# jjfiv/fastrank

Measured on AMD Instinct MI355X. Metric: coordinate-ascent NDCG@10 evals/sec on MSLR-WEB30K shape, higher is better.
Workload: dtype f64; 1 GPU; synthetic MSLR-WEB30K shape: 3800000 docs x 136 features x 31000 queries, coordinate ascent NDCG@10, 32 restarts/GPU x 25 steps/coord (configs[2]); restarts_total=32, parallelism=restart-sharded x1 (dataset replicated), launcher=single process

## Files before the change

fastrank_amd/csrc/capi.cpp:

```cpp
#include <atomic>
#include <limits>
#include <chrono>
#include <cstdio>
#include <cstdlib>
#include <cstring>
#include <fstream>

#include "../../include/fastrank.h"
#include "host.hpp"
#include "loader.hpp"
#include "explain_host.hpp"
#include "lambdamart.hpp"
#include "rf_train.hpp"

using fr::FrError;
using frjson::Value;

struct CDataset {
    std::shared_ptr<fr::DatasetView> view;
};
struct CModel {
    fr::Model actual;
};
struct CQRel {
// ... 1224 lines not shown
        auto holder = std::make_unique<FrTrainer>();
        holder->t0 = std::chrono::steady_clock::now();
        holder->t = std::make_unique<fr::CATrainer>(ds.view, std::move(ev), rq.ca, restart_begin, restart_end);
        holder->core = ds.view->core;
        h = holder.release();
    });
    if (st) {
        if (error_out) *error_out = st; else free((void*)st);
        return nullptr;
    }
    return h;
}

void* fr_ca_begin_query_shard(const void* train_request_json, const CDataset* dataset, uint64_t total_queries,
                              fr_allreduce_sum_fn allreduce, void* ctx, const void** error_out) {
    if (error_out) *error_out = nullptr;
    FrTrainer* h = nullptr;
    const void* st = status_call([&]() {
        const CDataset& ds = require_dataset(dataset);
        ParsedRequest rq = parse_train_request(accept_str("train_request_json", train_request_json));
        if (rq.learner != Learner::CoordinateAscent) fr::fail_str("fr_ca_begin_query_shard: only CoordinateAscent");
        if (!allreduce) fr::fail_str("fr_ca_begin_query_shard: allreduce callback is null!");
        std::lock_guard<std::mutex> lk(api_mu_of(ds));
        fr::Evaluator ev = fr::make_evaluator(*ds.view, rq.measure, rq.has_qrel ? &rq.qrel : nullptr);
        if (total_queries == 0) fr::fail_str("assertion failed: !data.queries().is_empty()");
        fr::QueryShard shard;
        shard.total_queries = total_queries;
        shard.allreduce = [allreduce, ctx](double* v, size_t n) {
            if (allreduce(ctx, v, n) != 0) fr::fail_str("query-shard allreduce callback failed");
        };
        auto holder = std::make_unique<FrTrainer>();
        holder->t0 = std::chrono::steady_clock::now();
        holder->t = std::make_unique<fr::CATrainer>(ds.view, std::move(ev), rq.ca, 0u, rq.ca.num_restarts, std::move(shard));
        holder->core = ds.view->core;
        h = holder.release();
    });
    if (st) {
        if (error_out) *error_out = st; else free((void*)st);
        return nullptr;
    }
    return h;
}

const void* fr_ca_step(void* trainer, uint64_t max_ticks, uint64_t* ticks_done, int* finished) {
    return status_call([&]() {
        if (!trainer) fr::fail_str("trainer pointer is null!");
        FrTrainer* h = (FrTrainer*)trainer;
        std::lock_guard<std::mutex> lk(h->core->api_mu);
        uint64_t n = 0;
        const bool alive = h->t->run(max_ticks, &n);
        if (ticks_done) *ticks_done = n;
        if (finished) *finished = (!alive || h->t->done()) ? 1 : 0;
    });
}

const void* fr_ca_state(void* trainer) {
    return json_call([&]() {
        if (!trainer) fr::fail_str("trainer pointer is null!");
        FrTrainer* h = (FrTrainer*)trainer;
        std::lock_guard<std::mutex> lk(h->core->api_mu);
        h->t->stats().seconds = std::chrono::duration<double>(std::chrono::steady_clock::now() - h->t0).count();
        Value o = Value::object();
        o.set("restarts", restarts_to_json(h->t->results()));
        o.set("stats", stats_to_json(h->t->stats()));
        o.set("finished", Value::boolean(h->t->done()));
        return frjson::dump(o);
    });
}

void fr_ca_free(void* trainer) { delete (FrTrainer*)trainer; }

const void* fr_ca_capture(void* trainer, int on) {
    return status_call([&]() {
        if (!trainer) fr::fail_str("trainer pointer is null!");
        FrTrainer* h = (FrTrainer*)trainer;
        std::lock_guard<std::mutex> lk(h->core->api_mu);
        h->t->capture(on != 0);
        if (!on) h->capture_blob.clear();
    });
}

const void* fr_ca_capture_take(void* trainer, const void* table, void* out, size_t out_bytes) {
    return json_call([&]() {
        if (!trainer) fr::fail_str("trainer pointer is null!");
        FrTrainer* h = (FrTrainer*)trainer;
        std::lock_guard<std::mutex> lk(h->core->api_mu);
        Value o = Value::object();
        if (table) {
            const std::string name = accept_str("table", table);
            if (name != "blob") fr::fail_str("fr_ca_capture_take: no table named " + name);
            if (out_bytes != h->capture_blob.size() || (!out && out_bytes))
                fr::fail_str("fr_ca_capture_take: the blob holds " + std::to_string(h->capture_blob.size()) + " bytes, the buffer " + std::to_string(out_bytes));
            if (out_bytes) std::memcpy(out, h->capture_blob.data(), out_bytes);
            o.set("bytes", Value::uint(out_bytes));
            h->capture_blob.clear();
            h->capture_blob.shrink_to_fit();
            return frjson::dump(o);
        }
        std::vector<frdev::LsCapture> log;
        h->t->take_capture(&log);
        std::vector<unsigned char>& blob = h->capture_blob;
        blob.clear();
        auto put = [&blob](const auto& v) {
            using T = typename std::remove_reference_t<decltype(v)>::value_type;
            blob.resize((blob.size() + 7) & ~size_t(7));
            Value r = Value::object();
            r.set("off", Value::uint(blob.size()));
            r.set("n", Value::uint(v.size()));
            const size_t at = blob.size();
            blob.resize(at + v.size() * sizeof(T));
            if (!v.empty()) std::memcpy(blob.data() + at, v.data(), v.size() * sizeof(T));
            return r;
        };
        Value events = Value::array();
        for (const frdev::LsCapture& e : log) {
            Value ev = Value::object();
            if (e.store) {
                ev.set("type", Value::string("store"));
                ev.set("slot", Value::sint(e.slot));
                ev.set("v", put(e.v));
                events.push(std::move(ev));
                continue;
            }
            static const char* const kinds[] = {"topk", "rr", "fullrank"};
            ev.set("type", Value::string("tick"));
            ev.set("ctx", Value::sint(e.ctx));
            ev.set("kind", Value::string(kinds[e.kind]));
            ev.set("measure", Value::sint(e.measure));
            ev.set("depth", Value::sint(e.depth));
            Value groups = Value::array();
            for (const frdev::LineGroup& lg : e.groups) {
                Value g = Value::object();
                g.set("feature", Value::uint(lg.feature));
                g.set("weights", put(lg.weights));
                g.set("candidates", put(lg.candidates));
                g.set("resident_slot", Value::sint(lg.resident_slot));
                g.set("resident_owner", Value::uint(lg.resident_owner));
                g.set("has_update", Value::boolean(lg.has_update));
                g.set("upd_feature", Value::uint(lg.upd_feature));
                g.set("params", put(std::vector<double>{lg.resident_norm, lg.resident_base_f, lg.resident_err, lg.upd_norm, lg.upd_base_f, lg.upd_cand}));
                groups.push(std::move(g));
            }
            ev.set("groups", std::move(groups));
            ev.set("gorder", put(e.gorder));
            ev.set("nverify", Value::uint(e.nverify));
            ev.set("approx", Value::boolean(e.approx));
            ev.set("resident", Value::boolean(e.resident));
            ev.set("ready", Value::boolean(e.ready));
            Value inst = Value::object();
            if (e.kind == 0) {
                inst.set("k", Value::sint(e.kbucket));
                inst.set("xs_used", Value::sint(e.xs_used));
                inst.set("xs_pinned", Value::boolean(e.xs_pinned));
            } else {
                inst.set("classes", put(e.classes));
            }
            inst.set("dup", Value::boolean(e.dup));
            ev.set("inst", std::move(inst));
            ev.set("redo", put(e.redo));
            ev.set("redo_groups", Value::uint(e.redo_groups));
            ev.set("means", put(e.means));
            ev.set("nq", Value::uint(e.nq));
            ev.set("ldm", Value::uint(e.ldm));
            ev.set("np", Value::uint(e.np));
            ev.set("has_matrix", Value::boolean(e.has_matrix));
            ev.set("matrix", put(e.matrix));
            ev.set("res_slots", put(e.res_slots));
            ev.set("res", put(e.res));
            events.push(std::move(ev));
        }
        o.set("events", std::move(events));
        o.set("bytes", Value::uint(blob.size()));
        return frjson::dump(o);
    });
}

const CResult* fr_select_model(const void* restarts_json, int output_ensemble) {
    return c_call<CModel>([&]() {
        std::vector<fr::RestartResult> hist = restarts_from_json_text(accept_str("restarts_json", restarts_json));
        std::stable_sort(hist.begin(), hist.end(),
                         [](const fr::RestartResult& a, const fr::RestartResult& b) { return a.restart_id < b.restart_id; });
        return new_model([&] { return fr::ca_select(hist, output_ensemble != 0); });
    });
}

const void* fr_last_train_stats(void) {
    return json_call([&]() {
        std::lock_guard<std::mutex> slk(g_stats_mu);
        Value o = stats_to_json(g_last_stats);
        if (!g_last_per_device.empty()) {
            Value a = Value::array();
            for (const fr::TrainStats& st : g_last_per_device) a.push(stats_to_json(st));
            o.set("per_device", std::move(a));
        }
        if (!g_last_lambdamart.is_null()) o.set("lambdamart", g_last_lambdamart);
        return frjson::dump(o);
    });
}

const void* fr_debug_tree_plan(void) {
    return json_call([&]() {
        const frdev::TreePlan p = frdev::last_tree_plan();
        Value o = Value::object();
        if (p.path == frdev::TreePlan::NONE) {
            o.set("path", Value::null());
            return frjson::dump(o);
        }
        o.set("path", Value::string(p.path == frdev::TreePlan::RANK ? "rank" : p.path == frdev::TreePlan::LDS ? "lds" : "l2"));
        o.set("cache_hit", Value::boolean(p.cache_hit));
        if (p.path == frdev::TreePlan::LDS) o.set("docs", Value::uint(p.docs)), o.set("parts", Value::uint(p.parts));
        if (p.path == frdev::TreePlan::L2) o.set("rows_in_lds", Value::boolean(p.rows_in_lds));
        if (p.path == frdev::TreePlan::RANK) o.set("nslots", Value::uint(p.nslots)), o.set("nrounds", Value::uint(p.nrounds));
        if (p.path != frdev::TreePlan::L2) {
            Value a = Value::array();
            for (const auto& b : p.batches) {
                Value pair = Value::array();
                pair.push(Value::uint(b.first)), pair.push(Value::uint(b.second));
                a.push(std::move(pair));
            }
            o.set("batches", std::move(a));
        }
        return frjson::dump(o);
    });
}

const void* fr_predict_scores_dense(const CModel* model, const CDataset* dataset, double* out, size_t out_len) {
    return status_call([&]() {
        const CModel& m = require_model(model);
        const CDataset& ds = require_dataset(dataset);
        std::lock_guard<std::mutex> lk(api_mu_of(ds));
        fr::DatasetView& view = *ds.view;
        if (view.instances.empty()) return;
        frdev::DeviceDataset& dev = view.device();
        fr::score_model(view, m.actual);
        std::string err;
        if (!dev.download_scores(0, out, out_len, &err)) fr::fail_str(err);
    });
}

namespace {

frdev::ExDocs explain_docs(fr::DatasetView& view) {
    frdev::DeviceDataset::TileForm tf;
    std::string err;
    if (!view.device().tile_form(&tf, &err)) fr::fail_str(err);
    if (tf.nonfinite) fr::fail_str("explain: the dataset holds inf or NaN feature values");
    frdev::ExDocs docs;
    docs.xb = tf.xb, docs.dq = (uint32_t)tf.dq, docs.d = (uint32_t)tf.d, docs.device = tf.device;
    docs.pos.reserve(tf.n), docs.ids.reserve(tf.n);
    for (size_t p = 0; p < tf.np; p++)
        if (tf.perm_host[p] != 0xFFFFFFFFu) docs.pos.push_back((uint32_t)p), docs.ids.push_back(tf.perm_host[p]);
    return docs;
}

size_t explain_budget() {
    const size_t free_b = frdev::device_free_bytes(), margin = (size_t)256 << 20;
    size_t budget = free_b > margin ? free_b - margin : 0;
    if (free_b == 0) budget = std::numeric_limits<size_t>::max();
    if (const char* e = std::getenv("FR_EXPLAIN_MAX_BYTES")) budget = std::min<size_t>(budget, (size_t)std::strtoull(e, nullptr, 10));
    return budget;
}

struct ExplainJob {
    fr::ExplainModel em;
    fr::ExplainPlan plan;
    frdev::ExDocs docs;
    std::vector<uint32_t> view_feats;
    std::vector<int64_t> out_col;
    frdev::ExTimes cover_t;
};

ExplainJob explain_prepare(const CModel& m, const CDataset& ds, const CDataset* bg) {
    ExplainJob job;
    job.em = fr::explain_model(m.actual);
    fr::DatasetView& view = *ds.view;
    fr::DatasetView& bview = bg ? *bg->view : view;
    if (bview.instances.empty()) fr::fail_str("explain: the background dataset holds no instance");
    job.view_feats = view.features;
    std::sort(job.view_feats.begin(), job.view_feats.end());
    if (view.instances.empty()) return job;
    job.docs = explain_docs(view);
    for (uint32_t f : job.em.feats) {
        const auto it = std::lower_bound(job.view_feats.begin(), job.view_feats.end(), f);
        const bool listed = it != job.view_feats.end() && *it == f;
        if (!listed && f < job.docs.d)
            fr::fail_str("explain: the model splits on feature " + std::to_string(f) + ", which the dataset's matrix holds but this feature sample does not list");
        job.out_col.push_back(listed ? (int64_t)(it - job.view_feats.begin()) : -1);
    }
    const frdev::ExWalk walk = fr::explain_walk(job.em);
    std::vector<uint32_t> counts;
    std::string err;
    if (&bview == &view) {
        if (!frdev::explain_covers(job.docs, walk, &counts, &job.cover_t, &err)) fr::fail_str(err);
    } else {
        const frdev::ExDocs bdocs = explain_docs(bview);
        if (bdocs.device != job.docs.device) fr::fail_str("explain: the background dataset lives on another device");
        if (!frdev::explain_covers(bdocs, walk, &counts, &job.cover_t, &err)) fr::fail_str(err);
    }
    job.plan = fr::explain_plan(job.em, counts, job.docs.d);
    return job;
}

Value explain_status(const ExplainJob& job, const frdev::ExTimes& t) {
    Value o = Value::object(), ids = Value::array(), sc = Value::array();
    for (uint32_t f : job.view_feats) ids.push(Value::uint(f));
    std::vector<uint64_t> counts(job.view_feats.size(), 0);
    for (size_t k = 0; k < job.out_col.size(); k++)
        if (job.out_col[k] >= 0) counts[(size_t)job.out_col[k]] = job.em.split_counts[k];
    for (uint64_t c : counts) sc.push(Value::uint(c));
    o.set("feature_ids", std::move(ids));
    o.set("split_counts", std::move(sc));
    o.set("expected_value", Value::number(job.plan.bias));
    o.set("trees", Value::uint(job.em.trees.size()));
    o.set("leaf_paths", Value::uint(job.plan.tab.value.size()));
    o.set("max_path", Value::uint(job.plan.tab.max_path));
    o.set("documents", Value::uint(job.docs.pos.size()));
    o.set("cover_ms", Value::number(job.cover_t.kernel_ms));
    o.set("kernel_ms", Value::number(t.kernel_ms));
    o.set("copy_ms", Value::number(t.copy_ms));
    return o;
}
// ... 717 lines not shown
```

fastrank_amd/csrc/device.hpp:

```cpp
#pragma once
#include <algorithm>
#include <cstddef>
#include <cstdint>
#include <memory>
#include <string>
#include <utility>
#include <vector>

#include "dataset_layout.hpp"

namespace frdev {

const char* path_env(const char* name);
inline const char* pricing_env(const char* name) {
#ifdef FR_PRICING
    return path_env(name);
#else
    (void)name;
    return nullptr;
#endif
}

enum Measure : int { M_NDCG = 0, M_AP = 1, M_RR = 2 };
constexpr int LM_OBJECTIVE_XENDCG = 3;

inline double resident_err_refresh(uint32_t d, double T) { return 1.1 * (double)(d + 1) * 0x1p-53 * T; }
inline double resident_err_update(double err, double norm, double T) { return 1.002 * err / norm + 8.0 * 0x1p-53 * T * (1.0 + 1e-6); }
inline double resident_eps_extra(double err, double norm, double T) { return 1.01 * err / norm + 10.0 * 0x1p-53 * T; }

enum : int {
    FLAG_NAN_SCORE = 1,
    FLAG_ACTUAL_GT_IDEAL = 2,
};

struct FlatTrees {
    std::vector<int32_t> fid, lhs, rhs;
    std::vector<double> split;
    std::vector<int32_t> root;
    std::vector<double> weight;
    bool raw_single = false;
};

struct TreePlan {
    enum Path { NONE, RANK, LDS, L2 };
    Path path = NONE;
    bool cache_hit = false;
    bool rows_in_lds = false;
    uint32_t docs = 0, parts = 0;
    uint32_t nslots = 0, nrounds = 0;
    std::vector<std::pair<uint32_t, uint32_t>> batches;
};
TreePlan last_tree_plan();

struct LineGroup {
    uint32_t feature = 0;
    std::vector<double> weights;
    std::vector<double> candidates;
    int resident_slot = -1;
    uint64_t resident_owner = 0;
    double resident_norm = 1.0, resident_base_f = 0.0, resident_err = 0.0;
    bool has_update = false;
    uint32_t upd_feature = 0;
    double upd_norm = 1.0, upd_base_f = 0.0, upd_cand = 0.0;
};

struct LsCapture {
    bool store = false;
    int slot = -1;
    std::vector<double> v;
    int ctx = 0, kind = 0, measure = 0;
    int64_t depth = 0;
    std::vector<LineGroup> groups;
    std::vector<uint32_t> gorder;
    size_t nverify = 0;
    bool approx = false, resident = false, ready = false;
    int kbucket = 0, xs_used = 0;
    bool xs_pinned = false, dup = false;
    std::vector<uint32_t> classes;
    std::vector<uint32_t> redo;
    uint32_t redo_groups = 0;
    std::vector<double> means;
    bool has_matrix = false;
    size_t nq = 0, ldm = 0, np = 0;
    std::vector<double> matrix;
    std::vector<int> res_slots;
    std::vector<double> res;
};

struct KernelStat {
    std::string name;
    uint64_t launches = 0;
    double total_ms = 0.0;
};

class DeviceDataset {
  public:
    static std::shared_ptr<DeviceDataset> create(const HostCSR& csr, std::string* err);
    static std::shared_ptr<DeviceDataset> create_view(const std::shared_ptr<DeviceDataset>& parent, const HostCSR& csr,
                                                      const std::vector<uint32_t>& parent_query, std::string* err);
    static std::shared_ptr<DeviceDataset> replicate(const std::shared_ptr<DeviceDataset>& src, int device, std::string* err);
    int device_ordinal() const;
    bool shares_parent_matrix() const;
    ~DeviceDataset();

    size_t n() const;
    size_t d() const;
    size_t nq() const;
    size_t max_query_len() const;
    size_t hbm_bytes() const;

    bool score_linear(size_t B, const double* weights, std::string* err);
    bool score_single_feature(uint32_t fid, double dir, std::string* err);
    bool score_trees(const FlatTrees& trees, std::string* err);
    bool ensemble_begin(std::string* err);
    bool ensemble_accumulate(double w, std::string* err);
    bool ensemble_finish(std::string* err);

    bool download_scores(size_t b, double* out_by_instance, size_t out_len, std::string* err);

    bool metric_from_scores(int measure, int64_t depth, const double* norms, size_t B,
                            bool want_rank, std::string* err);
    bool download_per_query(size_t B, double* out , std::string* err);
    bool download_rank(uint32_t* out_instance_ids , std::string* err);
    bool reduce_means(size_t ncols, double* out_means, std::string* err);
    void set_sums_only(bool on);
    bool subset_means_set(const std::vector<uint32_t>& a, const std::vector<uint32_t>& b, std::string* err);
    bool reduce_subset_means(double out_means[2], std::string* err);
    void subset_means_end();

    enum LsPath : int { LS_NONE = 0, LS_TOPK = 1, LS_FULLRANK = 2 };
    LsPath linesearch_path(int measure, int64_t depth) const;
    static constexpr int LINESEARCH_CONTEXTS = 4;
    struct LsCounts {
        unsigned long long pairs = 0, redone = 0;
    };
    bool linesearch_submit(int ctx, int measure, int64_t depth, const double* norms, const std::vector<LineGroup>& groups,
                           std::string* err);
    bool linesearch_collect(int ctx, std::vector<double>* means, LsCounts* counts, std::string* err);
    bool linesearch(int measure, int64_t depth, const double* norms, const std::vector<LineGroup>& groups,
                    std::vector<double>* means, LsCounts* counts, std::string* err);
    uint64_t resident_reserve(size_t slots, std::string* err);
    bool resident_store_from_scores(uint64_t owner, size_t slot, size_t b, std::string* err, const double* v = nullptr);
    void capture_enable(bool on);
    void capture_note_store(size_t slot, const double* v);
    void capture_take(std::vector<LsCapture>* out);
    const std::vector<double>& column_absmax() const;
    unsigned long long exact_fallbacks() const;
    void routing_counters(unsigned long long* exact_groups, unsigned long long* redo_entries) const;
    void chain_counters(unsigned long long* runs, unsigned long long* visits, unsigned long long* ranked_on = nullptr,
                        unsigned long long* ranked_off = nullptr) const;
    void audit_counters(unsigned long long* values, unsigned long long* mismatches) const;
    bool download_last_matrix(std::vector<double>* out, size_t* ldm, std::string* err);

    struct RfActive { uint32_t tree, key, n; };
    struct RfCand { double position, importance; uint32_t ids_i, flags, pos_l, pos_r; double sum_l, sum_r; };
    struct RfSplit { int32_t fslot; uint32_t pos, left, right; };
    bool rf_set_presence(const uint32_t* bits_by_instance, size_t words, size_t n_instances, std::string* err);
    bool rf_begin(const std::vector<uint32_t>& root_off, const std::vector<uint32_t>& root_ids, uint32_t nf,
                  const std::vector<uint32_t>& feats, std::string* err, const uint32_t* positions = nullptr,
                  bool lambda_targets = false);
    bool rf_positions(const std::vector<uint32_t>& root_ids, uint32_t* positions , std::string* err);
    bool rf_root_outputs(std::vector<double>* out, std::string* err);
    bool rf_level(const std::vector<RfActive>& active, const std::vector<uint32_t>& slot_of_key, uint32_t k, int method,
                  uint32_t min_leaf, std::vector<RfCand>* cands, std::vector<float>* label_minmax, std::string* err);
    bool rf_split(const std::vector<RfSplit>& splits, std::vector<double>* child_out, std::string* err);
    void rf_end();
    size_t rf_bytes_per_item() const { return 41; }

    struct LambdaPass {
        const unsigned char* query_flags = nullptr;
        bool flags_unchanged = false;
        uint32_t truncation_level = 0;
        bool lambda_norm = false;
        int objective = 0;
        uint64_t xe_key = 0;
    };
    bool lambda_gradients(const double* norms, int64_t depth, double sigma, const LambdaPass& pass, std::string* err);
    bool lambda_download_positions(std::vector<double>* lambda, std::vector<double>* weight, std::string* err);
    bool lambda_download(double* lambda_by_instance, double* weight_by_instance, size_t out_len, std::string* err,
                         const unsigned char* query_flags = nullptr);

    bool dart_begin(size_t rows, uint64_t* cache_bytes, std::string* err);
    bool dart_fill(size_t row, const double* leaf_values, size_t n_leaves, std::string* err);
    bool dart_rescore(const double* weights, size_t n_weights, const uint32_t* trees, size_t n_trees, std::string* err);
    bool dart_download_row(size_t row, uint16_t* out_by_instance, size_t out_len, std::string* err);
    void dart_end();

    struct HistNode { uint32_t slot, begin, end; };
    struct HistSplit { uint32_t begin, end, fslot, edge, nl; };
    struct HistSub { uint32_t parent, small, large; };
    struct HistBounds { double lo, hi; };
    struct HistSearch {
        uint32_t min_leaf; bool newton; int s_l, s_w; double lambda_l2, min_sum_hessian, min_split_gain; bool monotone;
        double lambda_l1 = 0.0, max_delta_step = 0.0, path_smooth = 0.0;
        bool reg() const { return lambda_l1 != 0.0 || max_delta_step != 0.0 || path_smooth != 0.0; }
    };
    struct HistRegNode { double lo, hi, parent; uint32_t has_parent, pad; };
    struct HistCand { double imp; long long ql, qtot, wl, wtot; uint32_t edge, nl, valid, fi; };
    bool hist_bins(const uint32_t* positions, size_t n, const std::vector<uint32_t>& feats, uint32_t k, bool* built, std::string* err);
    bool hist_edges(std::vector<float>* edges, std::vector<uint32_t>* nedges, std::string* err);
    bool hist_download_bins(uint8_t* out , size_t len, std::string* err);
    bool hist_sample(const unsigned char* query_flags, uint32_t n_t, const uint32_t* fsel, size_t f_t, std::string* err,
                     bool keep_queries = false);
    bool hist_goss(const double* lam_list, uint32_t n_top, double p, double amp, uint64_t tree_key, uint32_t* n_g, uint64_t* tau,
                   std::string* err);
    bool hist_goss_download(uint32_t* list, uint8_t* top, size_t len, std::string* err);
    bool hist_quantise(const double* lam_list, const double* wt_list, int* s_l, int* s_w, bool* all_zero, std::string* err);
    bool hist_quantq(uint32_t bits, uint64_t tree_key, int* d, int* d_w, std::string* err);
    bool hist_quantq_download(int32_t* q, uint32_t* w, size_t len, std::string* err);
    bool hist_root_download(uint32_t* cnt, long long* sum, long long* wsum, size_t cells, std::string* err);
    bool hist_root(bool newton, std::string* err);
    bool hist_search(const std::vector<HistNode>& nodes, const HistSearch& how, const std::vector<HistBounds>* bounds,
                     std::vector<HistCand>* best, std::string* err, const std::vector<HistRegNode>* reg = nullptr);
    bool hist_monotone(const int* signs, size_t features, std::string* err);
    struct HistSymBest { double key; uint32_t edge, valid; };
    bool hist_search_symmetric(const std::vector<HistNode>& nodes, const HistSearch& how, std::vector<HistSymBest>* best, std::string* err);
    bool hist_symmetric_apply(const std::vector<HistNode>& nodes, const HistSearch& how, uint32_t fi, uint32_t edge, std::vector<HistCand>* out,
                              std::string* err);
    bool hist_split(const std::vector<HistSplit>& splits, const std::vector<HistNode>& builds, const std::vector<HistSub>& subs,
                    uint32_t next_slots, bool newton, std::string* err);
    bool hist_leaf_sums(const std::vector<HistNode>& leaves, std::vector<long long>* qw , std::string* err);
    void hist_end();
    bool hist_leaf_begin(uint32_t slots, const HistSearch& how, HistCand* root, std::string* err);
    static constexpr uint32_t HIST_NO_SLOT = 0xffffffffu;
    struct HistLeafStep { HistSplit split; uint32_t parent_slot, small_slot; bool search_lhs, search_rhs; HistBounds bounds[2] = {}; double parent_out = 0.0; };
    bool hist_leaf_step(const HistLeafStep& step, const HistSearch& how, HistCand pick[2], std::string* err);

    struct TileForm {
        const float* xb = nullptr;
        size_t np = 0, dq = 0, d = 0, n = 0;
        int device = 0;
        bool nonfinite = false;
        const uint32_t* perm_host = nullptr;
    };
    bool tile_form(TileForm* out, std::string* err);

    int take_flags();

    std::vector<std::pair<std::string, uint64_t>> debug_form_scalars() const;
// ... 39 lines not shown
```

fastrank_amd/csrc/device_dataset.inc:

```

static constexpr int LS_CONTEXTS = DeviceDataset::LINESEARCH_CONTEXTS;

static double fv_class_cost(int ci) {
    static const int sort_ce[] = {63, 191, 384, 543, 849, 1056}, merge_ce[] = {32, 80, 144, 192, 304, 336};
    const uint32_t nl = FV_CLASSES[ci].nl, pl = FV_CLASSES[ci].pl;
    const int ni = (int)nl / 16 - 1;
    uint32_t rounds = 0;
    while ((1u << rounds) < pl) rounds++;
    double c = 2.0 * nl + 2.0 * sort_ce[ni] + 5.0 * nl + (double)nl * pl;
    for (uint32_t r = 1; r <= rounds; r++) c += 5.0 * r * nl + 2.0 * merge_ce[ni];
    static const double lane_penalty[] = {1.0, 1.1, 1.25, 1.6, 2.0, 2.4};
    return c * pl * lane_penalty[rounds];
}

static int fv_class_of(uint32_t len) {
    static const bool pow2_only = [] {
        const char* e = frdev::pricing_env("FR_FV_CLASSES");
        return e != nullptr && std::strcmp(e, "pow2") == 0;
    }();
    int best = -1;
    double best_cost = 0.0;
    for (int ci = 0; ci < FV_NCLASSES; ci++) {
        const uint32_t nl = FV_CLASSES[ci].nl, pl = FV_CLASSES[ci].pl, npad = nl * pl;
        if (npad < len) continue;
        if (pow2_only && ((npad & (npad - 1)) != 0 || (nl != 64 && pl != 1))) continue;
        const double c = fv_class_cost(ci);
        if (best < 0 || c < best_cost) best = ci, best_cost = c;
    }
    return best < 0 ? FV_NCLASSES - 1 : best;
}

void fullrank_class_of(uint32_t len, uint32_t* nl, uint32_t* pl) {
    const int ci = fv_class_of(len > 2048 ? 2048u : len);
    *nl = FV_CLASSES[ci].nl;
    *pl = FV_CLASSES[ci].pl;
}

std::vector<SizeClass> fv_build_classes(const std::vector<uint32_t>& qlen, std::vector<uint32_t>* list) {
    std::vector<int> cls_of_len(2049, -1);
    return bucket_queries(qlen, [&](uint32_t len) {
        const uint32_t l = len > 2048 ? 2048 : len;
        if (cls_of_len[l] < 0) cls_of_len[l] = fv_class_of(l);
        return cls_of_len[l];
    }, list);
}

static_assert(WT == WALK_TILE && LS_KT == DCG_RANKS && IDX_INVALID == NO_DOCUMENT, "the kernels' constants are the host layout's (dataset_layout.hpp)");

struct DatasetDesc {
    size_t n = 0, d = 0, nq = 0, np = 0, dq = 0, maxlen = 0, nruns = 0;
    bool nonfinite = false;
    bool labels_small_int = false;
    std::vector<double> colmax;
    int verify_xs = 1;
    std::vector<uint32_t> perm_host;
    std::vector<uint32_t> qstart_h, qlen_h, qnpos_h, qnneg_h;
    std::vector<uint32_t> wt_start_h;
    size_t nwt = 0;
    std::vector<double> colstd;
    std::vector<uint8_t> colmode;
    std::vector<ColStats> colstats_h;
    uint32_t key_bits = 0, key_cls_bits = 0;
    uint64_t dup_groups = 0;
    std::vector<SizeClass> size_classes;
    std::vector<SizeClass> fv_classes;
    uint64_t relmask = 0;
    size_t ncls = 0, tablen = 0;
};

struct StreamSignal {
    std::mutex mu;
    std::condition_variable cv;
    bool done = false, ok = true;
    void set(bool good) {
        {
            std::lock_guard<std::mutex> lk(mu);
            if (!good) ok = false;
            done = true;
        }
        cv.notify_all();
    }
    bool wait() {
        std::unique_lock<std::mutex> lk(mu);
        cv.wait(lk, [&] { return done; });
        return ok;
    }
};

struct DeviceDataset::Impl : DatasetDesc {
    struct TickStage {
        size_t G = 0, dp = 0;
        size_t o_count = 0, o_gredo = 0, o_gthr = 0, o_gmode = 0, o_rank = 0, o_gfeat = 0, o_gncand = 0, o_slot = 0, o_updf = 0, o_gcand = 0, o_eps2 = 0, o_par = 0, o_gw = 0, total = 0;
    };
    enum LsKind { LSK_TOPK, LSK_RR, LSK_FV };
    struct LsCtx {
        hipStream_t stream = nullptr;
        PinnedBuf tick_h, tick_res;
        DevBuf<unsigned char> tick_d;
        DevBuf<double> M, means, partial;
        DevBuf<uint32_t> redo;
        DevBuf<int> flags;
        template <typename T> T* th(size_t off) { return reinterpret_cast<T*>(tick_h.p + off); }
        template <typename T> T* td(size_t off) { return reinterpret_cast<T*>(tick_d.p + off); }
        bool pending = false, approx = false;
        bool ready = false;
        LsKind kind = LSK_TOPK;
        TickStage ts;
        LSArgs a;
        RRArgs ra;
        FSArgs fsa;
        RMArgs rma;
        DevBuf<double> fv_rows;
        size_t ldm = 0, maxc = 0, lds = 0;
        int64_t depth = 0;
        int measure = 0;
        int xs_used = 1;
        bool xs_pinned = false;
        bool audit = false;
        std::vector<LineGroup> agroups;
        unsigned redo_grid = 512, redo_grid_used = 512;
        size_t nverify = 0;
        std::vector<uint32_t> gorder, gredo_h;
        std::vector<int> gslot;
        std::vector<LineGroup> pgroups;
        std::vector<double> exact_means;
        LsCounts counts;
        bool resident = false, dup = false;
        int kbucket = 0;
        std::vector<LineGroup> cgroups;
    };
    LsCtx ls[LS_CONTEXTS + 1];
    hipEvent_t res_ready = nullptr;
    bool res_ready_set = false;
    const double* last_M = nullptr;
    DevBuf<uint32_t> sub_idx;
    DevBuf<double> sub_partial, sub_means;
    uint32_t sub_na = 0, sub_nb = 0;
    bool ls_submit(LsCtx& c, int path, int measure, int64_t depth, const double* norms, const std::vector<LineGroup>& groups,
                   std::string* err);
    struct LsTick { const std::vector<LineGroup>& groups; const double* norms; size_t nV; bool resident, any_update; };
    bool submit_topk(LsCtx& c, const LsTick& t, std::string* err);
    bool submit_rr(LsCtx& c, const LsTick& t, std::string* err);
    bool submit_fv(LsCtx& c, const LsTick& t, std::string* err);
    bool exact_instead(LsCtx& c, const LsTick& t, std::string* err);
    bool submit_queued(LsCtx& c, const LsTick& t, size_t nverify, std::string* err);
    bool ls_collect(LsCtx& c, std::vector<double>* means, std::string* err);
    bool topk_policy(LsCtx& c, uint32_t nredo, uint32_t nslices, std::string* err);
    bool ls_exact(LsCtx& c, int measure, int64_t depth, const double* norms, const std::vector<LineGroup>& groups, std::string* err);
    bool exact_kernels(const std::vector<LineGroup>& groups, int measure, int64_t depth, size_t maxc, double* M, int* flags, std::string* err);
    bool fr_audit(LsCtx& c, std::string* err);
    bool cap_on = false;
    std::vector<LsCapture> cap_log;
    const LsCtx* cap_outer = nullptr;
    bool capture_tick(LsCtx& c, const std::vector<double>& means, uint32_t nredo, std::string* err);
    bool ls_means(LsCtx& c, std::string* err);
    bool tick_begin(LsCtx& c, const std::vector<LineGroup>& groups, std::string* err);
    bool tick_upload(LsCtx& c, bool with_eps2, std::string* err);
    bool tick_finish(LsCtx& c, size_t ldm, std::vector<double>* means, uint32_t* nredo, std::string* err, uint32_t* npairs = nullptr,
                     std::vector<uint32_t>* by_group = nullptr);
    bool stage_resident(LsCtx& c, const std::vector<LineGroup>& groups, bool* any_update_out);
    bool compute_eps2(const std::vector<LineGroup>& groups, bool resident, uint32_t cls_bits, bool bare_admission = false, bool key_relative = false);
    double eps_gamma = 0.0;
    bool update_resident(LsCtx& c, size_t g_base, size_t ng, std::string* err);
    void flip_resident(const std::vector<LineGroup>& groups);
    bool redo_launch(LsCtx& c, uint32_t off, const uint32_t* count_dev, uint32_t n, std::string* err);
    FSArgs scores_args(const uint32_t* gfeat, const double* gw, const double* gcand, double* rows, int* flags, size_t gc) const;
    RMArgs rank_args(const double* rows, const uint32_t* gncand, double* M, int* flags, size_t gc, size_t ldm, int measure, int64_t depth) const;
    void topk_args(LsCtx& c, size_t G) const;
    RRArgs rr_args(LsCtx& c, size_t G) const;
    FVArgs fv_args(LsCtx& c, size_t G, uint32_t cls_bits, uint32_t dup_bits) const;
    int device = 0;
    hipStream_t stream = nullptr;
    std::vector<double> eps2_host;
    DevBuf<double> res;
    std::vector<uint8_t> res_half;
    uint64_t res_owner = 0;
    LsPolicy pol;
    unsigned long long approx_pairs = 0, approx_redo = 0;
    unsigned long long approx_redo_entries = 0;
    unsigned long long chain_runs = 0, chain_visits = 0;
    unsigned long long audit_values = 0, audit_mismatches = 0;
    DevBuf<double> audit;
    DevBuf<unsigned long long> audit_cnt;
    DevBuf<int> audit_flags;
    unsigned long long exact_fallbacks = 0;
    std::shared_ptr<DeviceDataset> parent;
    DevBuf<uint32_t> run_lo;
    DevBuf<uint32_t> vtiles;
    size_t nvtiles = 0;
    PosMap posmap() const { return PosMap{nvtiles ? vtiles.p : nullptr, (uint32_t)nvtiles, (uint32_t)np}; }
    size_t pos_threads() const { return nvtiles ? nvtiles * 64 : np; }
    DevBuf<uint8_t> xslot;
    DevBuf<uint16_t> segtab;
    DevBuf<uint32_t> wt_start;
    DevBuf<uint32_t> run_wt0;
    DevBuf<uint8_t> wofs;
    DevBuf<uint32_t> wlist;
    size_t nwlist = 0;
    DevBuf<uint8_t> rslot;
    hipError_t open_streams(bool* at_event, StreamSignal* main_stream = nullptr);
    bool open_streams(std::string* err);
    static bool upload_tiles(Impl& m, const HostCSR& csr, bool timing, StreamSignal& main_stream, std::string* terr);
    bool build_order_tables(std::string* err);
    DevBuf<float> xcol;
    bool build_columns(std::string* err);
    DevBuf<uint16_t> gkey;
    DevBuf<float> xb, gain;
    DevBuf<double> gexp, disc;
    DevBuf<uint32_t> qstart, qlen, qtight, perm, rank, run_q0, run_q1, run_pos, run_docs, run_order, gcls, qlist;
    DevBuf<uint32_t> fv_qlist;
    DevBuf<uint32_t> qnpos, qnneg, sort_idx;
    DevBuf<double> sort_keys;
    DevBuf<double> termtab, rows;
    DevBuf<double> dcgtab;
    DevBuf<int> flags;
    DevBuf<unsigned long long> dbgc;
    DevBuf<double> scores, acc, weights, M, means, partial, norms, gw, gcand;
    DevBuf<uint32_t> gfeat, gncand;
    DevBuf<TreeNodeDev> nodes;
    DevBuf<int32_t> roots;
    DevBuf<double> tweights;
    struct RfState {
        DevBuf<uint32_t> roff, pos, node_of, feats, slot_of_key, act_tree, act_n, vals_a, vals_b;
        DevBuf<uint64_t> act_off, act_first, keys_a, keys_b;
        DevBuf<float> sg, sv, sg_o, sv_o, label, gain_r;
        DevBuf<unsigned char> temp;
        DevBuf<RfCandDev> cands;
        DevBuf<RfSplitDev> splits;
        DevBuf<double> child;
        std::vector<uint32_t> roff_h;
        std::vector<uint32_t> pos_of_id;
        std::mutex pos_mu;
        uint32_t T = 0, nf = 0, total = 0;
        uint32_t A = 0;
        uint64_t items = 0, node_items = 0;
        bool sorted_in_b = false;
        uint64_t prev_items = 0;
        uint32_t prev_A = 0;
        DevBuf<uint32_t> act_tree_o, act_n_o;
        DevBuf<uint32_t> pres;
        uint32_t pw = 0;
        DevBuf<uint64_t> act_off_o;
        DevBuf<uint64_t> tile_first_o;
        DevBuf<uint32_t> tile_cnt;
        DevBuf<unsigned char> side, side_r;
        std::vector<uint32_t> prev_act_n;
        uint32_t splits_for_A = 0;
        const float* targets = nullptr;
    } rf;
    void rf_args(RFArgs& a);
    struct LmState {
        bool built = false;
        DevBuf<uint32_t> off, pos, qorder;
        DevBuf<double> lam, wt;
        DevBuf<float> target;
        DevBuf<unsigned char> slab;
        uint32_t n_lds = 0, max_len = 0;
        std::vector<uint32_t> order_h, qsel_h;
        uint32_t sel_long = 0;
        bool qsel_valid = false;
        DevBuf<uint32_t> qsel;
        DevBuf<double> asum;
    } lm;
    bool lm_build(std::string* err);
    struct DartState {
        DevBuf<uint16_t> leaf;
        DevBuf<double> vals, w;
        DevBuf<uint32_t> voff, trees;
        DevBuf<int> bad;
        std::vector<double> vals_h, w_h;
        std::vector<uint32_t> voff_h, trees_h;
        size_t rows = 0, filled = 0, stride = 0;
    } dart;
    struct HistState {
        uint32_t k = 0, n = 0, F = 0;
        uint32_t nt = 0, Ft = 0;
        bool q_sampled = false, f_sampled = false, qof_built = false, qof_ok = false;
        DevBuf<uint32_t> qof, root, fsel, total;
        DevBuf<uint8_t> qflag;
        bool g_on = false;
        uint32_t ng = 0;
// ... 1012 lines not shown
    const size_t ldm = c.ldm;
    if (!c.tick_res.ensure((ldm + mean_tail_words(ldm)) * sizeof(double), err)) return false;
    return launch_means(c.M.p, ldm, ldm, m.nq, m.sums_only, c.partial, c.means, c.stream, err, c.td<unsigned long long>(c.ts.o_count),
                        c.flags.p, reinterpret_cast<double*>(c.tick_res.p), c.kind == LSK_TOPK ? c.td<uint32_t>(c.ts.o_gredo) : nullptr);
}

bool DeviceDataset::Impl::tick_finish(LsCtx& c, size_t ldm, std::vector<double>* means, uint32_t* nredo, std::string* err,
                                      uint32_t* npairs, std::vector<uint32_t>* by_group) {
    Impl& m = *this;
    const size_t tail = ldm * sizeof(double);
    hipStream_t st = c.stream;
    FR_HIP(hipStreamSynchronize(st));
    means->resize(ldm);
    std::memcpy(means->data(), c.tick_res.p, tail);
    unsigned long long words[2] = {0, 0};
    std::memcpy(words, c.tick_res.p + tail, sizeof(words));
    *nredo = (uint32_t)words[0];
    if (npairs) *npairs = (uint32_t)(words[0] >> 32);
    if (by_group) {
        by_group->resize(2 * (ldm / 64));
        std::memcpy(by_group->data(), c.tick_res.p + tail + 16, 2 * (ldm / 64) * sizeof(uint32_t));
    }
    const int v = (int)(unsigned int)words[1];
    if (v) {
        m.host_flags |= v;
        FR_HIP(hipMemsetAsync(c.flags.p, 0, sizeof(int), st));
        FR_HIP(hipStreamSynchronize(st));
    }
    return true;
}
bool DeviceDataset::Impl::stage_resident(LsCtx& c, const std::vector<LineGroup>& groups, bool* any_update_out) {
    Impl& m = *this;
    const TickStage& ts = c.ts;
    LSArgs& a = c.a;
    const size_t G = groups.size();
    bool resident = G > 0, any_update = false;
    for (const LineGroup& lg : groups) {
        resident = resident && lg.resident_owner == m.res_owner && m.res_owner != 0 && lg.resident_slot >= 0 &&
                   (size_t)lg.resident_slot < m.res_half.size();
        any_update = any_update || lg.has_update;
    }
    a.res_cur = m.res.p;
    a.np = (uint32_t)m.np;
    a.rs_slot = nullptr;
    a.rs_par = nullptr;
    a.rs_updf = nullptr;
    a.xcol = m.xcol.p;
    if (resident) {
        int32_t* rs_slot = c.th<int32_t>(ts.o_slot);
        double* rs_par = c.th<double>(ts.o_par);
        uint32_t* rs_updf = c.th<uint32_t>(ts.o_updf);
        for (size_t g = 0; g < G; g++) {
            const LineGroup& lg = groups[g];
            rs_slot[g] = (int32_t)(lg.resident_slot * 2 + m.res_half[lg.resident_slot]);
            rs_par[g * 6 + 0] = 1.0 / lg.resident_norm;
            rs_par[g * 6 + 1] = lg.resident_base_f;
            rs_par[g * 6 + 2] = lg.has_update ? 1.0 : 0.0;
            rs_par[g * 6 + 3] = 1.0 / lg.upd_norm;
            rs_par[g * 6 + 4] = lg.upd_base_f;
            rs_par[g * 6 + 5] = lg.upd_cand;
            rs_updf[g] = lg.upd_feature;
        }
        a.rs_slot = c.td<int32_t>(ts.o_slot);
        a.rs_par = c.td<double>(ts.o_par);
        a.rs_updf = c.td<uint32_t>(ts.o_updf);
    }
    *any_update_out = any_update;
    return resident;
}

bool DeviceDataset::Impl::compute_eps2(const std::vector<LineGroup>& groups, bool resident, uint32_t cls_bits, bool bare_admission, bool key_relative) {
    Impl& m = *this;
    const size_t G = groups.size();
    std::vector<double>& eps2 = m.eps2_host;
    eps2.assign(G * 64, 0.0);
    const double dfac = (key_relative && resident) ? (double)(m.d + 2) : 2.5 * (double)(m.d + 1);
    const double gamma = (dfac * std::ldexp(1.0, -53) + (bare_admission ? 3.0 : 2.0) * std::ldexp(1.0, (int)cls_bits - 52)) * (1.0 + 1e-6);
    bool ok = true;
    for (size_t g = 0; g < G; g++) {
        const LineGroup& lg = groups[g];
        double T = 0.0;
        for (size_t j = 0; j < m.d; j++)
            if (j != lg.feature) T += std::fabs(lg.weights[j]) * m.colmax[j];
        double extra = 0.0;
        if (resident) {
            T += std::fabs(lg.resident_base_f) * m.colmax[lg.feature];
            extra = resident_eps_extra(lg.resident_err, lg.resident_norm, T);
            if (!(lg.resident_norm > 0.0) || !(extra < 1e290)) ok = false;
        }
        for (size_t c = 0; c < lg.candidates.size(); c++) {
            const double Tc = T + std::fabs(lg.candidates[c]) * m.colmax[lg.feature];
            if (!(Tc < 1e290)) ok = false;
            const double floor_abs = 1e-300 + std::fabs(lg.candidates[c]) * std::ldexp(1.0, (int)cls_bits - 1070);
            eps2[g * 64 + c] = key_relative ? 2.0 * (gamma * 2.0 * T + extra + floor_abs) : 2.0 * (gamma * Tc + extra + floor_abs);
        }
    }
    m.eps_gamma = gamma;
    return ok;
}

bool DeviceDataset::Impl::update_resident(LsCtx& c, size_t g_base, size_t ng, std::string* err) {
    Impl& m = *this;
    LSArgs x = c.a;
    x.g_base = (uint32_t)g_base;
    x.posmap = m.posmap();
    {
        ProfScope ps("resident_update_kernel", c.stream);
        resident_update_kernel<<<dim3((unsigned)((m.pos_threads() + 255) / 256), (unsigned)ng), 256, 0, c.stream>>>(x);
    }
    FR_HIP(hipGetLastError());
    return true;
}


void DeviceDataset::Impl::flip_resident(const std::vector<LineGroup>& groups) {
    Impl& m = *this;
    std::vector<char> flipped(m.res_half.size(), 0);
    for (const LineGroup& lg : groups)
        if (lg.has_update && !flipped[lg.resident_slot]) {
            m.res_half[lg.resident_slot] ^= 1;
            flipped[lg.resident_slot] = 1;
        }
}

template <int K, int CT>
static void launch_linesearch(const LSArgs& a, unsigned nblocks, size_t lds, hipStream_t st) {
    linesearch_ndcg_kernel<K, CT, 16><<<dim3(nblocks), dim3(WAVE), lds, st>>>(a);
}

template <int K>
static void dispatch_ct(const LSArgs& a, unsigned nblocks, size_t maxc, size_t lds, hipStream_t st) {
    if (maxc <= 4) launch_linesearch<K, 4>(a, nblocks, lds, st);
    else if (maxc <= 16) launch_linesearch<K, 16>(a, nblocks, lds, st);
    else if (maxc <= 32) launch_linesearch<K, 32>(a, nblocks, lds, st);
    else if (maxc <= 51) launch_linesearch<K, 51>(a, nblocks, lds, st);
    else launch_linesearch<K, 64>(a, nblocks, lds, st);
}

static void dispatch_exact(const LSArgs& a, int64_t depth, unsigned nblocks, size_t maxc, size_t lds, hipStream_t st) {
    if (a.work_list != nullptr) {
        maxc = std::min<size_t>(maxc, 16);
        nblocks *= 4;
    }
    if (depth <= 5) dispatch_ct<5>(a, nblocks, maxc, lds, st);
    else if (depth <= 10) dispatch_ct<10>(a, nblocks, maxc, lds, st);
    else dispatch_ct<20>(a, nblocks, maxc, lds, st);
}

static unsigned redo_grid_env() {
    const char* e = frdev::path_env("FR_REDO_GRID");
    return e ? (unsigned)std::min<long>(std::max<long>(std::atol(e), 64), 1 << 20) : 0u;
}

template <int K>
static void launch_verify(const LSArgs& a, bool resident, bool dupk, int xs, unsigned nruns8, size_t G, size_t dp, size_t tab_lds_kt, hipStream_t st) {
    const size_t tab_lds = tab_lds_kt / (LS_KT + 1) * (K + 1);
    if (resident) {
        const dim3 grid((unsigned)(nruns8 * G));
        if (dupk) {
            if (xs <= 1) linesearch_verify_kernel<K, 1, true, 1, true><<<grid, dim3(WAVE), tab_lds, st>>>(a);
            else if (xs == 2) linesearch_verify_kernel<K, 1, true, 2, true><<<grid, dim3(WAVE), tab_lds, st>>>(a);
            else if (xs == 3 || K < 10) linesearch_verify_kernel<K, 1, true, 3, true><<<grid, dim3(WAVE), tab_lds, st>>>(a);
            else linesearch_verify_kernel<K, 1, true, (K < 10 ? 3 : 4), true><<<grid, dim3(WAVE), tab_lds, st>>>(a);
        } else if (xs <= 1) linesearch_verify_kernel<K, 1, true><<<grid, dim3(WAVE), tab_lds, st>>>(a);
        else if (xs == 2) linesearch_verify_kernel<K, 1, true, 2><<<grid, dim3(WAVE), tab_lds, st>>>(a);
        else if (xs == 3 || K < 10) linesearch_verify_kernel<K, 1, true, 3><<<grid, dim3(WAVE), tab_lds, st>>>(a);
        else linesearch_verify_kernel<K, 1, true, (K < 10 ? 3 : 4)><<<grid, dim3(WAVE), tab_lds, st>>>(a);
    } else {
        const dim3 grid((unsigned)(nruns8 * ((G + 1) / 2)));
        linesearch_verify_kernel<K, 2, false><<<grid, dim3(WAVE), 2 * dp * sizeof(double) + tab_lds, st>>>(a);
    }
}

uint64_t DeviceDataset::resident_reserve(size_t slots, std::string* err) {
    Impl& m = *impl_;
    std::lock_guard<std::mutex> lk(m.mu);
    if (!m.bind(err)) return 0;
    m.res_owner++;
    m.verify_xs = std::max(1, m.verify_xs - 1);
    m.res_half.clear();
    if (m.xcol.p == nullptr) {
        if (err) *err = "resident_reserve: the dataset has no column-major copy";
        return 0;
    }
    m.pol.reset(slots);
    {
        std::string* e2 = err;
        auto ensure = [&]() -> bool { return m.res.ensure(slots * 2 * m.np, e2); };
        if (!ensure()) return 0;
    }
    m.res_half.assign(slots, 0);
    if (m.xslot.p != nullptr) {
        std::string e2;
        if (m.rslot.ensure(slots * m.np, &e2)) {
            rslot_identity_kernel<<<dim3(1024), dim3(256), 0, m.stream>>>(m.rslot.p, m.wofs.p, m.np, slots * m.np);
            if (hipGetLastError() != hipSuccess) m.rslot.release();
        } else {
            (void)hipGetLastError();
        }
    }
    return m.res_owner;
}

bool DeviceDataset::resident_store_from_scores(uint64_t owner, size_t slot, size_t b, std::string* err, const double* v) {
    Impl& m = *impl_;
    std::lock_guard<std::mutex> lk(m.mu);
    if (err) err->clear();
    if (owner != m.res_owner) return false;
    if (!m.bind(err)) return false;
    if (slot >= m.res_half.size() || b >= m.scores_slots) {
        if (err) *err = "resident_store_from_scores: slot out of range";
        return false;
    }
    FR_HIP(hipMemcpyAsync(m.res.p + (slot * 2 + m.res_half[slot]) * m.np, m.scores.p + b * m.np, m.np * sizeof(double),
                          hipMemcpyDeviceToDevice, m.stream));
    FR_HIP(hipEventRecord(m.res_ready, m.stream));
    m.res_ready_set = true;
    m.pol.new_sums(slot);
    if (m.cap_on) {
        LsCapture e;
        e.store = true;
        e.slot = (int)slot;
        if (v) e.v.assign(v, v + m.d);
        m.cap_log.push_back(std::move(e));
    }
    return true;
}

void DeviceDataset::capture_enable(bool on) {
    std::lock_guard<std::mutex> lk(impl_->mu);
    impl_->cap_on = on;
    if (!on) impl_->cap_log.clear();
    for (Impl::LsCtx& c : impl_->ls) std::vector<LineGroup>().swap(c.cgroups);
}

void DeviceDataset::capture_note_store(size_t slot, const double* v) {
    std::lock_guard<std::mutex> lk(impl_->mu);
    if (!impl_->cap_on) return;
    LsCapture e;
    e.store = true;
    e.slot = (int)slot;
    e.v.assign(v, v + impl_->d);
    impl_->cap_log.push_back(std::move(e));
}

void DeviceDataset::capture_take(std::vector<LsCapture>* out) {
    std::lock_guard<std::mutex> lk(impl_->mu);
    out->clear();
    out->swap(impl_->cap_log);
}

const std::vector<double>& DeviceDataset::column_absmax() const { return impl_->colmax; }

void DeviceDataset::audit_counters(unsigned long long* values, unsigned long long* mismatches) const {
    std::lock_guard<std::mutex> lk(impl_->mu);
    *values = impl_->audit_values;
    *mismatches = impl_->audit_mismatches;
}

unsigned long long DeviceDataset::exact_fallbacks() const {
    std::lock_guard<std::mutex> lk(impl_->mu);
    return impl_->exact_fallbacks;
}

void DeviceDataset::chain_counters(unsigned long long* runs, unsigned long long* visits, unsigned long long* ranked_on,
                                   unsigned long long* ranked_off) const {
    std::lock_guard<std::mutex> lk(impl_->mu);
    *runs = impl_->chain_runs;
    *visits = impl_->chain_visits;
    if (ranked_on) *ranked_on = impl_->pol.rank_slots_on;
    if (ranked_off) *ranked_off = impl_->pol.rank_slots_off;
}

void DeviceDataset::routing_counters(unsigned long long* exact_groups, unsigned long long* redo_entries) const {
    std::lock_guard<std::mutex> lk(impl_->mu);
    *exact_groups = impl_->pol.exact_groups;
    *redo_entries = impl_->approx_redo_entries;
}

static void launch_scores(const FSArgs& a, size_t maxc, unsigned nblocks, size_t lds, hipStream_t st) {
    if (maxc <= 16) linesearch_scores_kernel<16, 16><<<dim3(nblocks), dim3(WAVE), lds, st>>>(a);
    else if (maxc <= 51) linesearch_scores_kernel<51, 16><<<dim3(nblocks), dim3(WAVE), lds, st>>>(a);
    else linesearch_scores_kernel<64, 16><<<dim3(nblocks), dim3(WAVE), lds, st>>>(a);
}

FSArgs DeviceDataset::Impl::scores_args(const uint32_t* gf, const double* w, const double* cand, double* rows, int* fl, size_t gc) const {
    FSArgs a{};
    a.xb = (const float4*)xb.p;
    a.run_pos = run_pos.p;
    a.run_docs = run_docs.p;
    a.run_order = run_order.p;
    a.gfeat = gf;
    a.gw = w;
    a.gcand = cand;
    a.rows = rows;
    a.flags = fl;
    a.dq = (uint32_t)dq;
    a.d = (uint32_t)d;
    a.nruns = (uint32_t)nruns;
    a.GC = (uint32_t)gc;
    a.np = (uint32_t)np;
    return a;
}

RMArgs DeviceDataset::Impl::rank_args(const double* rows, const uint32_t* gnc, double* out, int* fl, size_t gc, size_t ldm, int measure,
                                      int64_t depth) const {
    RMArgs a{};
    a.rows = rows;
    a.qstart = qstart.p;
    a.qlen = qlen.p;
    a.qnpos = qnpos.p;
    a.qnneg = qnneg.p;
    a.gcls = gcls.p;
    a.termtab = termtab.p;
    a.norms = norms.p;
    a.gncand = gnc;
    a.M = out;
    a.flags = fl;
    a.GC = (uint32_t)gc;
    a.np = (uint32_t)np;
// ... 256 lines not shown
            return false;
        }
        maxc = std::max(maxc, lg.candidates.size());
    }
    if (&c == &m.ls[LS_CONTEXTS]) c.stream = m.stream;
    c.kind = path == LS_TOPK ? LSK_TOPK : (measure == M_RR ? LSK_RR : LSK_FV);
    c.ldm = G * 64;
    c.maxc = maxc;
    c.depth = depth;
    c.measure = measure;
    c.approx = c.ready = false;
    c.resident = c.dup = false;
    c.kbucket = 0;
    c.nverify = 0;
    c.gorder.clear();
    c.counts = LsCounts{};
    if (m.cap_on) c.cgroups = groups_in;
    if (G == 0) {
        c.pending = true;
        return true;
    }
    const bool topk = c.kind == LSK_TOPK;
    if (topk) {
        if (m.nq * G >= (size_t(1) << 28)) {
            if (err) *err = "linesearch: too many (query, group) pairs for one launch";
            return false;
        }
        if (!c.M.ensure(m.nq * c.ldm, err) || !c.redo.ensure(m.nq * G, err)) return false;
    }
    const bool exact_only = std::getenv("FR_LS_EXACT") != nullptr;
    c.audit = std::getenv("FR_VERIFY_AUDIT") != nullptr;
    bool can_verify = !exact_only && m.colmax.size() == m.d;
    if (c.kind != LSK_RR) can_verify = can_verify && m.ncls <= 256;
    if (c.kind == LSK_FV)
        can_verify = can_verify && frdev::path_env("FR_FV_OFF") == nullptr && (measure == M_NDCG ? m.termtab.cap > 0 : m.ncls <= 31);
    if (!can_verify && !topk) return m.ls_exact(c, measure, depth, norms, groups_in, err);
    if (c.kind != LSK_RR) {
        if (!m.norms.ensure(m.nq, err)) return false;
        const uint64_t tok = groups_in[0].resident_owner;
        if (!(tok != 0 && tok == m.norms_token && norms == m.norms_token_ptr)) {
            const bool fresh = !(m.norms_cache.size() == m.nq && std::memcmp(m.norms_cache.data(), norms, m.nq * sizeof(double)) == 0);
            if (!m.upload_norms(norms, err)) return false;
            if (fresh) FR_HIP(hipStreamSynchronize(m.stream));
            m.norms_token = tok;
            m.norms_token_ptr = norms;
        }
    }
    size_t nV = can_verify ? G : 0;
    const std::vector<LineGroup>* gp = &groups_in;
    if (topk && can_verify && m.res_owner != 0) {
        const size_t nE = m.pol.route(G, [&](size_t g) { return groups_in[g].resident_owner == m.res_owner ? (long)groups_in[g].resident_slot : -1L; });
        nV = G - nE;
        if (nE > 0 && nV > 0) {
            c.gorder.resize(G);
            size_t iv = 0, ie = nV;
            for (size_t g = 0; g < G; g++) c.gorder[m.pol.routed[g] ? ie++ : iv++] = (uint32_t)g;
            c.pgroups.clear();
            for (size_t k = 0; k < G; k++) c.pgroups.push_back(groups_in[c.gorder[k]]);
            gp = &c.pgroups;
        }
    }
    if (topk && nV == 0) m.exact_fallbacks++;
    if (!m.tick_begin(c, *gp, err)) return false;
    c.a = LSArgs{};
    LsTick t{*gp, norms, nV, false, false};
    t.resident = m.stage_resident(c, t.groups, &t.any_update);
    c.resident = t.resident;
    switch (c.kind) {
        case LSK_TOPK: return m.submit_topk(c, t, err);
        case LSK_RR: return m.submit_rr(c, t, err);
        case LSK_FV: return m.submit_fv(c, t, err);
    }
    return false;
}

bool DeviceDataset::Impl::submit_queued(LsCtx& c, const LsTick& t, size_t nverify, std::string* err) {
    Impl& m = *this;
    const size_t G = t.groups.size();
    const bool approx = nverify > 0;
    FR_HIP(hipGetLastError());
    if (!m.ls_means(c, err)) return false;
    if (t.resident) m.flip_resident(t.groups);
    c.gslot.assign(G, -1);
    if (t.resident)
        for (size_t k = 0; k < G; k++) c.gslot[k] = t.groups[k].resident_slot;
    c.agroups.clear();
    if (c.audit && approx && c.kind != LSK_TOPK) c.agroups.assign(t.groups.begin(), t.groups.end());
    c.approx = approx;
    c.nverify = nverify;
    c.pending = true;
    return true;
}

bool DeviceDataset::Impl::exact_instead(LsCtx& c, const LsTick& t, std::string* err) {
    Impl& m = *this;
    if (t.resident && t.any_update) {
        if (!m.update_resident(c, 0, t.groups.size(), err)) return false;
        m.flip_resident(t.groups);
    }
    FR_HIP(hipStreamSynchronize(c.stream));
    return m.ls_exact(c, c.measure, c.depth, t.norms, t.groups, err);
}

bool DeviceDataset::Impl::submit_topk(LsCtx& c, const LsTick& t, std::string* err) {
    Impl& m = *this;
    const std::vector<LineGroup>& groups = t.groups;
    const size_t G = groups.size(), dp = m.dq * 4, nruns8 = ((m.nruns + 7) / 8) * 8, maxc = c.maxc;
    const int64_t depth = c.depth;
    const bool resident = t.resident;
    const TickStage& ts = c.ts;
    size_t nV = t.nV;
    LSArgs& a = c.a;
    m.topk_args(c, G);
    static const int ls_debug = [] {
        const char* dbg = frdev::pricing_env("FR_LS_DEBUG");
        return dbg ? atoi(dbg) : 0;
    }();
    LS_DEBUG_SET(a, ls_debug);
    if (LS_DEBUG(a) & 16) FR_HIP(hipMemsetAsync(m.dbgc.p, 0, 4 * sizeof(unsigned long long), c.stream));
    if (nruns8 * G > 0x7fffffffull) {
        if (err) *err = "linesearch: grid too large";
        return false;
    }
    c.lds = 2 * dp * sizeof(double);
    bool approx = nV > 0 && (LS_DEBUG(a) & ~3) == 0;
    if (approx) approx = m.compute_eps2(groups, resident, m.key_bits, true, true);
    a.gamma = m.eps_gamma;
    const size_t tab_lds = (m.ncls + 1) * (size_t)(LS_KT + 1) * sizeof(double);
    if (approx && !resident && 2 * dp * sizeof(double) + tab_lds + 2 * (WAVE + 4) * sizeof(uint4) > 64 * 1024) approx = false;
    if (!approx && nV > 0) {
        m.exact_fallbacks++;
        nV = 0;
    }
    size_t nrank = 0;
    a.xslot = nullptr;
    if (approx && resident && m.xslot.p != nullptr && m.rslot.p != nullptr && m.colstd.size() == m.d) {
        static const double kappa = [] {
            const char* e = frdev::pricing_env("FR_ORDER_KAPPA");
            return e ? std::atof(e) : 1.0;
        }();
        static const unsigned period = [] {
            const char* e = frdev::pricing_env("FR_RANK_PERIOD");
            return e ? (unsigned)std::max(1, std::atoi(e)) : 16u;
        }();
        double* gthr = c.th<double>(ts.o_gthr);
        uint32_t* gmode = c.th<uint32_t>(ts.o_gmode);
        for (size_t g = 0; g < nV; g++) {
            gthr[g] = order_threshold(groups[g].weights, m.colstd, groups[g].feature, kappa);
            gmode[g] = m.colmode[groups[g].feature];
        }
        int32_t* rank = c.th<int32_t>(ts.o_rank);
        nrank = m.pol.plan_rank_refresh(nV, [&](size_t g) { return (size_t)groups[g].resident_slot; }, [&](size_t g) { return groups[g].has_update; },
                                        period, m.res_half, rank, rank + G);
        a.xslot = m.xslot.p;
        a.rslot = m.rslot.p;
        a.gthr = c.td<double>(ts.o_gthr);
        a.gmode = c.td<uint32_t>(ts.o_gmode);
    }
    if (!m.tick_upload(c, approx, err)) return false;
    if (!approx) {
        if (resident && t.any_update && !m.update_resident(c, 0, G, err)) return false;
        {
            ProfScope ps("linesearch_ndcg_kernel", c.stream);
            dispatch_exact(a, depth, (unsigned)(nruns8 * G), maxc, c.lds, c.stream);
        }
        return m.submit_queued(c, t, 0, err);
    }
    if (nrank > 0) {
        ProfScope ps("rslot_kernel", c.stream);
        const uint32_t* wl = m.nwlist ? m.wlist.p : nullptr;
        const unsigned nw = (unsigned)(m.nwlist ? m.nwlist : m.nwt);
        rslot_kernel<<<dim3((nw + 3) / 4), 256, 0, c.stream>>>(m.res.p, c.td<int32_t>(ts.o_rank), c.td<int32_t>(ts.o_rank) + G, (uint32_t)nrank,
                                                              a.rs_par, a.rs_updf, m.xcol.p, m.segtab.p, m.wt_start.p, wl, nw, (uint32_t)m.np, m.rslot.p);
        FR_HIP(hipGetLastError());
        if (c.audit) {
            if (!m.audit_cnt.ensure(1, err)) return false;
            FR_HIP(hipMemsetAsync(m.audit_cnt.p, 0, sizeof(unsigned long long), c.stream));
            const int32_t* rk = c.th<int32_t>(ts.o_rank);
            for (size_t k = 0; k < nrank; k++)
                order_audit_kernel<<<dim3((nw + 3) / 4), 256, 0, c.stream>>>(m.rslot.p + (size_t)(rk[k] >> 1) * m.np, m.segtab.p, m.wt_start.p, wl, nw, m.audit_cnt.p);
            for (size_t g = 0; g < nV; g++)
                order_audit_kernel<<<dim3((nw + 3) / 4), 256, 0, c.stream>>>(m.xslot.p + (size_t)groups[g].feature * m.np, m.segtab.p, m.wt_start.p, wl, nw, m.audit_cnt.p);
            unsigned long long bad = 0;
            FR_HIP(hipMemcpyAsync(&bad, m.audit_cnt.p, sizeof(bad), hipMemcpyDeviceToHost, c.stream));
            FR_HIP(hipStreamSynchronize(c.stream));
            m.audit_mismatches += bad;
        }
    }
    const char* xs_e = frdev::path_env("FR_VERIFY_XS");
    const int xs = std::min(xs_e ? std::atoi(xs_e) : m.verify_xs, verify_xs_cap(depth));
    c.xs_used = xs;
    c.xs_pinned = xs_e != nullptr;
    a.eps2 = c.td<double>(ts.o_eps2);
    a.G = (uint32_t)nV;
    const bool dupk = resident && m.key_bits > m.key_cls_bits;
    c.dup = dupk;
    {
        ProfScope ps("linesearch_verify_kernel", c.stream);
        if (depth <= 5) launch_verify<5>(a, resident, dupk, xs, (unsigned)nruns8, nV, dp, tab_lds, c.stream), c.kbucket = 5;
        else if (depth <= 10) launch_verify<10>(a, resident, dupk, xs, (unsigned)nruns8, nV, dp, tab_lds, c.stream), c.kbucket = 10;
        else launch_verify<20>(a, resident, dupk, xs, (unsigned)nruns8, nV, dp, tab_lds, c.stream), c.kbucket = 20;
    }
    FR_HIP(hipGetLastError());
    a.slice_count = c.td<uint32_t>(ts.o_count) + 1;
    const unsigned redo_pin = redo_grid_env();
    c.redo_grid_used = redo_pin ? redo_pin : c.redo_grid;
    if (!m.redo_launch(c, 0, c.td<uint32_t>(ts.o_count), c.redo_grid_used, err)) return false;
    if (nV < G) {
        if (t.any_update && !m.update_resident(c, nV, G - nV, err)) return false;
        LSArgs x = a;
        x.work_list = nullptr;
        x.work_count = nullptr;
        x.g_base = (uint32_t)nV;
        x.G = (uint32_t)(G - nV);
        ProfScope ps("linesearch_ndcg_kernel", c.stream);
        dispatch_exact(x, depth, (unsigned)(nruns8 * (G - nV)), maxc, c.lds, c.stream);
    }
    return m.submit_queued(c, t, nV, err);
}

bool DeviceDataset::Impl::submit_rr(LsCtx& c, const LsTick& t, std::string* err) {
    Impl& m = *this;
    const size_t G = t.groups.size();
    if (!t.resident) return m.ls_exact(c, c.measure, c.depth, t.norms, t.groups, err);
    bool approx = m.compute_eps2(t.groups, true, 0);
    if (approx && m.pol.take_skip()) m.exact_fallbacks++, approx = false;
    if (!m.tick_upload(c, approx, err)) return false;
    if (!approx) return m.exact_instead(c, t, err);
    if (!c.M.ensure(m.nq * c.ldm, err) || !c.redo.ensure(m.nq * G, err)) return false;
    RRArgs& ra = c.ra;
    ra = m.rr_args(c, G);
    {
        ProfScope ps("rr_verify_kernel", c.stream);
        FR_HIP(hipFuncSetAttribute((const void*)rr_verify_kernel, hipFuncAttributeMaxDynamicSharedMemorySize, 128 * 1024));
        for (size_t ci = m.size_classes.size(); ci-- > 0;) {
            const auto& sc = m.size_classes[ci];
            ra.qlist = m.qlist.p + sc.offset;
            rr_verify_kernel<<<dim3((unsigned)sc.count, (unsigned)G), WAVE, (size_t)sc.npad * sizeof(uint4), c.stream>>>(ra);
        }
    }
    FR_HIP(hipGetLastError());
    const unsigned redo_pin = redo_grid_env();
    c.redo_grid_used = redo_pin ? redo_pin : RR_REDO_GRID;
    if (!m.redo_launch(c, 0, c.td<uint32_t>(c.ts.o_count), c.redo_grid_used, err)) return false;
    return m.submit_queued(c, t, G, err);
}

bool DeviceDataset::Impl::submit_fv(LsCtx& c, const LsTick& t, std::string* err) {
    Impl& m = *this;
    const size_t G = t.groups.size();
    uint32_t cls_bits = 0;
    while ((size_t(1) << cls_bits) < m.ncls + 1) cls_bits++;
    const uint32_t dup_bits = (m.key_bits > m.key_cls_bits && cls_bits + (m.key_bits - m.key_cls_bits) <= 20) ? m.key_bits - m.key_cls_bits : 0u;
    bool approx = m.compute_eps2(t.groups, t.resident, cls_bits + dup_bits);
    if (approx && m.pol.take_skip()) m.exact_fallbacks++, approx = false;
    if (!m.tick_upload(c, approx, err)) return false;
    if (!approx) return m.exact_instead(c, t, err);
    if (!c.M.ensure(m.nq * c.ldm, err) || !c.redo.ensure(m.nq * G, err)) return false;
    const size_t slot_rows = ((m.maxlen + 63) / 64 + 1) * 64;
    if (!c.fv_rows.ensure((size_t)FV_REDO_GRID * slot_rows * 64, err)) return false;
    FVArgs fa = m.fv_args(c, G, cls_bits, dup_bits);
    c.dup = dup_bits != 0;
    {
        static const bool per_class = frdev::pricing_env("FR_FV_PROFILE") != nullptr;
        ProfScope ps_all(per_class ? "fullrank_verify_all" : "fullrank_verify_kernel", c.stream);
        for (size_t ci = m.fv_classes.size(); ci-- > 0;) {
            const auto& sc = m.fv_classes[ci];
            static std::vector<std::string> names = [] {
                std::vector<std::string> v;
                for (int i = 0; i < FV_NCLASSES; i++) v.push_back("fullrank_verify_kernel<" + std::to_string(FV_CLASSES[i].nl) + "x" + std::to_string(FV_CLASSES[i].pl) + ">");
                return v;
            }();
            std::unique_ptr<ProfScope> ps(per_class ? new ProfScope(names[sc.npad].c_str(), c.stream) : nullptr);
            fa.qlist = m.fv_qlist.p + sc.offset;
            if (!fv_launch_class(fa, (int)sc.npad, (unsigned)sc.count, (unsigned)G, (unsigned)c.maxc, c.stream)) {
                if (err) *err = "fullrank_verify_kernel: no instantiation for this size class";
                return false;
            }
        }
    }
    FR_HIP(hipGetLastError());
    FSArgs& fs = c.fsa;
    fs = m.scores_args(fa.gfeat, fa.gw, fa.gcand, c.fv_rows.p, c.flags.p, G);
    fs.qstart = m.qstart.p;
    fs.qlen = m.qlen.p;
    fs.G = (uint32_t)G;
    fs.slot_rows = (uint32_t)slot_rows;
    RMArgs& rm = c.rma;
    rm = m.rank_args(c.fv_rows.p, fa.gncand, c.M.p, c.flags.p, G, c.ldm, c.measure, c.depth);
    rm.G = (uint32_t)G;
    rm.slot_rows = (uint32_t)slot_rows;
    c.redo_grid_used = FV_REDO_GRID;
    if (!m.redo_launch(c, 0, c.td<uint32_t>(c.ts.o_count), FV_REDO_GRID, err)) return false;
    return m.submit_queued(c, t, G, err);
}

bool DeviceDataset::Impl::ls_exact(LsCtx& c, int measure, int64_t depth, const double* norms, const std::vector<LineGroup>& groups,
                                   std::string* err) {
    Impl& m = *this;
    if (&c != &m.ls[LS_CONTEXTS]) {
        c.pgroups.assign(groups.begin(), groups.end());
        for (LineGroup& lg : c.pgroups) lg.has_update = false;
        LsCtx& l = m.ls[LS_CONTEXTS];
        m.cap_outer = &c;
        const bool done = m.ls_submit(l, LS_FULLRANK, measure, depth, norms, c.pgroups, err) && m.ls_collect(l, &c.exact_means, err);
        m.cap_outer = nullptr;
        if (!done) return false;
        c.counts = l.counts;
        c.ready = c.pending = true;
        return true;
    }
    const size_t G = groups.size(), ldm = G * 64;
    std::vector<double>& means = c.exact_means;
    means.assign(ldm, 0.0);
    if (!m.M.ensure(m.nq * ldm, err) || !m.norms.ensure(m.nq, err) || !m.means.ensure(ldm, err)) return false;
    if (!m.upload_norms(norms, err)) return false;
    if (!m.exact_kernels(groups, measure, depth, c.maxc, m.M.p, m.flags.p, err)) return false;
    if (!launch_means(m.M.p, ldm, ldm, m.nq, m.sums_only, m.partial, m.means, m.stream, err)) return false;
    FR_HIP(hipMemcpyAsync(means.data(), m.means.p, ldm * sizeof(double), hipMemcpyDeviceToHost, m.stream));
    m.last_ldm = ldm;
    m.last_cols = ldm;
    m.last_M = m.M.p;
    if (!m.pull_flags(err)) return false;
    c.ready = c.pending = true;
    return true;
}

bool DeviceDataset::Impl::exact_kernels(const std::vector<LineGroup>& groups, int measure, int64_t depth, size_t maxc, double* M,
                                        int* flags, std::string* err) {
    Impl& m = *this;
    const size_t G = groups.size(), dp = m.dq * 4, ldm = G * 64;
    const size_t row_bytes = 64 * sizeof(double);
    size_t budget = m.rows.bytes();
    if (G * m.np * row_bytes > budget) {
        size_t free_b = 0, total_b = 0;
        (void)hipMemGetInfo(&free_b, &total_b);
        budget = std::max<size_t>(size_t(1) << 30, (free_b + m.rows.bytes()) / 2);
    }
    size_t GC = std::max<size_t>(1, std::min<size_t>(G, budget / (m.np * row_bytes)));
    if (!m.rows.ensure(m.np * GC * 64, err) || !m.gfeat.ensure(GC, err) || !m.gncand.ensure(GC, err) || !m.gw.ensure(GC * dp, err) ||
        !m.gcand.ensure(GC * 64, err))
        return false;
    for (size_t g0 = 0; g0 < G; g0 += GC) {
        const size_t gc = std::min(GC, G - g0);
        std::vector<uint32_t> gfeat(gc), gncand(gc);
        std::vector<double> gw(gc * dp, 0.0), gcand(gc * 64, 0.0);
        for (size_t g = 0; g < gc; g++) {
            const LineGroup& lg = groups[g0 + g];
            gfeat[g] = lg.feature;
            gncand[g] = (uint32_t)lg.candidates.size();
            std::memcpy(&gw[g * dp], lg.weights.data(), m.d * sizeof(double));
            std::memcpy(&gcand[g * 64], lg.candidates.data(), lg.candidates.size() * sizeof(double));
        }
        FR_HIP(hipMemcpyAsync(m.gfeat.p, gfeat.data(), gc * sizeof(uint32_t), hipMemcpyHostToDevice, m.stream));
        FR_HIP(hipMemcpyAsync(m.gncand.p, gncand.data(), gc * sizeof(uint32_t), hipMemcpyHostToDevice, m.stream));
        FR_HIP(hipMemcpyAsync(m.gw.p, gw.data(), gc * dp * sizeof(double), hipMemcpyHostToDevice, m.stream));
        FR_HIP(hipMemcpyAsync(m.gcand.p, gcand.data(), gc * 64 * sizeof(double), hipMemcpyHostToDevice, m.stream));
        FR_HIP(hipStreamSynchronize(m.stream));
        {
            ProfScope ps("linesearch_scores_kernel", m.stream);
            const FSArgs fa = m.scores_args(m.gfeat.p, m.gw.p, m.gcand.p, m.rows.p, flags, gc);
            launch_scores(fa, maxc, (unsigned)(((m.nruns + 7) / 8) * 8 * gc), 2 * dp * sizeof(double), m.stream);
        }
        FR_HIP(hipGetLastError());
        RMArgs ra = m.rank_args(m.rows.p, m.gncand.p, M, flags, gc, ldm, measure, depth);
        ra.col0 = (uint32_t)(g0 * 64);
        {
            ProfScope ps("rank_metric_kernel", m.stream);
            FR_HIP(hipFuncSetAttribute((const void*)rank_metric_kernel, hipFuncAttributeMaxDynamicSharedMemorySize,
                                       128 * 1024));
            for (size_t ci = m.size_classes.size(); ci-- > 0;) {
                const auto& sc = m.size_classes[ci];
                ra.qlist = m.qlist.p + sc.offset;
                dim3 grid((unsigned)sc.count, (unsigned)gc);
                const unsigned waves = (measure != M_NDCG && measure != M_AP) ? 1u
                                       : sc.npad <= 128 ? 1u : (sc.npad <= 256 ? 2u : (sc.npad <= 512 ? 4u : 8u));
                rank_metric_kernel<<<grid, WAVE * waves, (size_t)sc.npad * 64, m.stream>>>(ra);
            }
        }
        FR_HIP(hipGetLastError());
    }
    return true;
}

bool DeviceDataset::Impl::ls_collect(LsCtx& c, std::vector<double>* means, std::string* err) {
    Impl& m = *this;
    c.pending = false;
    if (c.ready) {
        *means = c.exact_means;
        if (m.cap_on) return m.capture_tick(c, *means, 0, err);
        return true;
    }
    const size_t ldm = c.ldm, G = ldm / 64;
    means->assign(ldm, 0.0);
    if (G == 0) return true;
    uint32_t nredo = 0, nslices = 0;
    std::vector<uint32_t>& by_group = c.gredo_h;
    if (!m.tick_finish(c, ldm, means, &nredo, err, &nslices, c.kind == LSK_TOPK ? &by_group : nullptr)) return false;
    LSArgs& a = c.a;
    if (c.approx) {
        const size_t nV = c.nverify;
        m.approx_pairs += m.nq * nV;
        m.approx_redo += nredo;
        c.counts.pairs += m.nq * nV;
        c.counts.redone += nredo;
        const unsigned grid = c.redo_grid_used;
        uint32_t again = 0;
        if (nredo > grid &&
            (!m.redo_launch(c, grid, nullptr, nredo - grid, err) || !m.ls_means(c, err) || !m.tick_finish(c, ldm, means, &again, err, &nslices)))
            return false;
        switch (c.kind) {
            case LSK_TOPK:
                if (!m.topk_policy(c, nredo, nslices, err)) return false;
                break;
            default:
                m.pol.observe_skip(nredo, m.nq, G);
                if (c.audit && !m.fr_audit(c, err)) return false;
                break;
        }
    }
    if (!c.gorder.empty()) {
        std::vector<double> tmp(*means);
        for (size_t k = 0; k < G; k++) std::memcpy(means->data() + (size_t)c.gorder[k] * 64, tmp.data() + k * 64, 64 * sizeof(double));
    }
    m.last_ldm = ldm;
    m.last_cols = ldm;
    m.last_M = c.M.p;
    if (LS_DEBUG(a) & 16) {
        unsigned long long cnt[4];
        FR_HIP(hipMemcpyAsync(cnt, m.dbgc.p, sizeof(cnt), hipMemcpyDeviceToHost, c.stream));
        FR_HIP(hipStreamSynchronize(c.stream));
        fprintf(stderr, "[FR_LS_DEBUG] docs=%llu rows=%llu (%.3f of docs) batches=%llu insertion_rows=%llu\n", cnt[3], cnt[0],
                (double)cnt[0] / (double)cnt[3], cnt[1], cnt[2]);
    }
    if (m.cap_on) return m.capture_tick(c, *means, c.approx ? nredo : 0, err);
    return true;
}

bool DeviceDataset::Impl::capture_tick(LsCtx& c, const std::vector<double>& means, uint32_t nredo, std::string* err) {
    Impl& m = *this;
    const bool lockstep = &c == &m.ls[LS_CONTEXTS];
    if (c.ready && !lockstep) return true;
    const LsCtx& who = (lockstep && m.cap_outer) ? *m.cap_outer : c;
    if (who.cgroups.size() * 64 != c.ldm) return true;
    LsCapture e;
    e.ctx = (int)(&who - m.ls);
    e.kind = (int)c.kind;
    e.measure = c.measure;
    e.depth = c.depth;
    e.groups = who.cgroups;
    const size_t G = e.groups.size();
    e.gorder = c.gorder;
    if (e.gorder.empty())
        for (size_t g = 0; g < G; g++) e.gorder.push_back((uint32_t)g);
    e.nverify = c.approx ? c.nverify : 0;
    e.approx = c.approx;
    e.resident = who.resident;
    e.ready = c.ready;
    hipStream_t st = c.ready ? m.stream : c.stream;
    if (c.kind == LSK_TOPK) {
        e.kbucket = c.kbucket;
        e.xs_used = c.kbucket ? c.xs_used : 0;
        e.xs_pinned = c.kbucket ? c.xs_pinned : false;
    } else if (c.approx) {
        if (c.kind == LSK_FV)
            for (const auto& sc : m.fv_classes) e.classes.insert(e.classes.end(), {FV_CLASSES[sc.npad].nl, FV_CLASSES[sc.npad].pl, sc.count});
        else
            for (const auto& sc : m.size_classes) e.classes.insert(e.classes.end(), {sc.npad, 1u, sc.count});
    }
    e.dup = c.dup;
    e.redo_groups = (uint32_t)(c.kind == LSK_TOPK ? c.nverify : G);
    if (c.approx && nredo > 0) {
        e.redo.resize(nredo);
        FR_HIP(hipMemcpyAsync(e.redo.data(), c.redo.p, nredo * sizeof(uint32_t), hipMemcpyDeviceToHost, st));
    }
    e.means = means;
    e.nq = m.nq;
    e.ldm = G * 64;
    e.np = m.np;
    const double* M = c.ready ? m.M.p : c.M.p;
    e.has_matrix = M != nullptr;
    if (e.has_matrix) {
        e.matrix.resize(e.nq * e.ldm);
        FR_HIP(hipMemcpyAsync(e.matrix.data(), M, e.matrix.size() * sizeof(double), hipMemcpyDeviceToHost, st));
    }
    if (e.resident) {
        for (const LineGroup& lg : e.groups) e.res_slots.push_back(lg.resident_slot);
        std::sort(e.res_slots.begin(), e.res_slots.end());
        e.res_slots.erase(std::unique(e.res_slots.begin(), e.res_slots.end()), e.res_slots.end());
        e.res.resize(e.res_slots.size() * m.np);
        for (size_t i = 0; i < e.res_slots.size(); i++) {
            const size_t slot = (size_t)e.res_slots[i];
            FR_HIP(hipMemcpyAsync(e.res.data() + i * m.np, m.res.p + (slot * 2 + m.res_half[slot]) * m.np, m.np * sizeof(double), hipMemcpyDeviceToHost, st));
        }
    }
    FR_HIP(hipStreamSynchronize(st));
    m.cap_log.push_back(std::move(e));
    return true;
}

bool DeviceDataset::Impl::fr_audit(LsCtx& c, std::string* err) {
    Impl& m = *this;
    const size_t nel = m.nq * c.ldm;
    if (!m.audit.ensure(nel, err) || !m.audit_cnt.ensure(1, err) || !m.audit_flags.ensure(1, err)) return false;
    FR_HIP(hipMemsetAsync(m.audit.p, 0xFF, nel * sizeof(double), m.stream));
    size_t ncells = 0;
    for (size_t g = 0; g < c.agroups.size(); g++) {
        const size_t nc = c.agroups[g].candidates.size();
        ncells += m.nq * nc;
        if (nc < 64)
            FR_HIP(hipMemcpy2DAsync(m.audit.p + g * 64 + nc, c.ldm * sizeof(double), c.M.p + g * 64 + nc, c.ldm * sizeof(double),
                                    (64 - nc) * sizeof(double), m.nq, hipMemcpyDeviceToDevice, m.stream));
    }
    FR_HIP(hipMemsetAsync(m.audit_flags.p, 0, sizeof(int), m.stream));
    if (!m.exact_kernels(c.agroups, c.measure, c.depth, c.maxc, m.audit.p, m.audit_flags.p, err)) return false;
    FR_HIP(hipMemsetAsync(m.audit_cnt.p, 0, sizeof(unsigned long long), m.stream));
    audit_compare_kernel<<<dim3(1024), dim3(256), 0, m.stream>>>(m.audit.p, c.M.p, nel, m.audit_cnt.p);
    FR_HIP(hipGetLastError());
    unsigned long long bad = 0;
    FR_HIP(hipMemcpyAsync(&bad, m.audit_cnt.p, sizeof(bad), hipMemcpyDeviceToHost, m.stream));
    FR_HIP(hipStreamSynchronize(m.stream));
    m.audit_values += ncells;
    m.audit_mismatches += bad;
    return true;
}

bool DeviceDataset::Impl::topk_policy(LsCtx& c, uint32_t nredo, uint32_t nslices, std::string* err) {
    Impl& m = *this;
    const size_t ldm = c.ldm, G = ldm / 64, nV = c.nverify;
    const std::vector<uint32_t>& by_group = c.gredo_h;
    LSArgs& a = c.a;
    c.redo_grid = next_redo_grid(c.redo_grid, c.redo_grid_used, nredo);
    m.approx_redo_entries += nslices;
    for (size_t k = 0; k < nV; k++) m.chain_runs += by_group[G + k];
    m.chain_visits += (unsigned long long)m.n * nV;
    {
        static const double t_off = [] {
            const char* e = frdev::pricing_env("FR_RANK_OFF_BELOW");
            return e ? std::atof(e) : RANK_OFF_BELOW;
        }();
        static const double t_on = [] {
            const char* e = frdev::pricing_env("FR_RANK_ON_ABOVE");
            return e ? std::atof(e) : RANK_ON_ABOVE;
        }();
        m.pol.observe_chain(nV, [&](size_t k) { return (long)c.gslot[k]; }, [&](size_t k) { return by_group[G + k]; }, m.n, t_off, t_on);
    }
    if (c.audit) {
        const size_t nel = m.nq * ldm;
        if (!m.audit.ensure(nel, err) || !m.audit_cnt.ensure(1, err)) return false;
        FR_HIP(hipMemcpyAsync(m.audit.p, c.M.p, nel * sizeof(double), hipMemcpyDeviceToDevice, c.stream));
        LSArgs x = a;
        x.work_list = nullptr;
        x.work_count = nullptr;
        x.g_base = 0;
        x.G = (uint32_t)G;
        dispatch_exact(x, c.depth, (unsigned)(((m.nruns + 7) / 8) * 8 * G), c.maxc, c.lds, c.stream);
        FR_HIP(hipMemsetAsync(m.audit_cnt.p, 0, sizeof(unsigned long long), c.stream));
        audit_compare_kernel<<<dim3(1024), dim3(256), 0, c.stream>>>(m.audit.p, c.M.p, nel, m.audit_cnt.p);
        unsigned long long bad = 0;
        FR_HIP(hipMemcpyAsync(&bad, m.audit_cnt.p, sizeof(bad), hipMemcpyDeviceToHost, c.stream));
        FR_HIP(hipStreamSynchronize(c.stream));
        m.audit_values += nel;
        m.audit_mismatches += bad;
    }
    m.pol.observe_redo(nV, [&](size_t k) { return (long)c.gslot[k]; }, [&](size_t k) { return by_group[k]; }, m.nq, c.xs_used, verify_xs_cap(c.depth),
                       c.xs_pinned, LS_DEBUG(a), m.verify_xs);
    return true;
}

bool DeviceDataset::linesearch_submit(int ctx, int measure, int64_t depth, const double* norms, const std::vector<LineGroup>& groups,
                                      std::string* err) {
    Impl& m = *impl_;
    std::lock_guard<std::mutex> lk(m.mu);
    if (!m.bind(err)) return false;
    if (ctx < 0 || ctx >= LS_CONTEXTS || m.ls[ctx].pending) {
        if (err) *err = "linesearch_submit: no such context, or a submitted line search was not collected";
        return false;
    }
    return m.ls_submit(m.ls[ctx], linesearch_path(measure, depth), measure, depth, norms, groups, err);
}

bool DeviceDataset::linesearch_collect(int ctx, std::vector<double>* means, LsCounts* counts, std::string* err) {
    Impl& m = *impl_;
    std::lock_guard<std::mutex> lk(m.mu);
    if (!m.bind(err)) return false;
    if (ctx < 0 || ctx >= LS_CONTEXTS || !m.ls[ctx].pending) {
        if (err) *err = "linesearch_collect: nothing was submitted on this context";
        return false;
    }
    if (!m.ls_collect(m.ls[ctx], means, err)) return false;
    if (counts) *counts = m.ls[ctx].counts;
    return true;
}

bool DeviceDataset::linesearch(int measure, int64_t depth, const double* norms, const std::vector<LineGroup>& groups,
                               std::vector<double>* means, LsCounts* counts, std::string* err) {
    Impl& m = *impl_;
    std::lock_guard<std::mutex> lk(m.mu);
    if (!m.bind(err)) return false;
    const LsPath path = linesearch_path(measure, depth);
    Impl::LsCtx& c = m.ls[path == LS_TOPK ? 0 : LS_CONTEXTS];
    if (c.pending) {
        if (err) *err = "linesearch: context 0 busy (collect the submitted line search first)";
        return false;
    }
    if (!m.ls_submit(c, path, measure, depth, norms, groups, err) || !m.ls_collect(c, means, err)) return false;
    if (counts) *counts = c.counts;
    return true;
}





#include "train_rf.inc"
#include "train_lambda.inc"
#include "train_dart.inc"
#include "train_hist.inc"
```

fastrank_amd/csrc/kernels_linesearch.inc:

```
struct LSArgs {
    const float4* xb;
    const uint32_t* gcls;
    const double* dcgtab;
    const uint32_t* qstart;
    const uint32_t* qlen;
    const uint32_t* run_q0;
    const uint32_t* run_q1;
    const uint32_t* run_pos;
    const uint32_t* run_lo;
    const uint32_t* run_docs;
    const uint32_t* run_order;
    const uint32_t* wt_start;
    const uint32_t* run_wt0;
    const double* norms;
    const double* disc;
    const uint32_t* gfeat;
    const double* gw;
    const double* gcand;
    const uint32_t* gncand;
    double* M;
    int* flags;
    unsigned long long* dbg_counters;
    const double* eps2;
    double gamma;
    unsigned long long* redo_count;
    uint32_t* redo_list;
    uint32_t* chain_count;
    const uint32_t* work_list;
    const uint32_t* work_count;
    uint32_t* slice_count;
    uint32_t g_base;
    uint32_t cls_mask;
    uint32_t cls_only_mask;
    const uint16_t* gkey;
    double* res_cur;
    const int32_t* rs_slot;
    const double* rs_par;
    const float* xcol;
    const uint32_t* rs_updf;
    const uint8_t* xslot;
    const uint8_t* rslot;
    const double* gthr;
    const uint32_t* gmode;
    uint32_t np;
    PosMap posmap;
    uint32_t dq, d, nruns, G, ldm;
    uint32_t ncls;
    int depth;
#ifdef FR_PRICING
    int debug;
#endif
};
#ifdef FR_PRICING
#define LS_DEBUG(A) ((A).debug)
#define LS_DEBUG_SET(A, V) ((A).debug = (V))
#else
#define LS_DEBUG(A) 0
#define LS_DEBUG_SET(A, V) ((void)(V))
#endif

constexpr int LS_ROWPAD = 65;
constexpr int LS_KT = 20;
#ifndef LS_WAVES_PER_SIMD
#define LS_WAVES_PER_SIMD 3
#endif

__device__ __forceinline__ uint64_t lane_range_mask(uint32_t lo, uint32_t hi) {
    const uint64_t up = (hi >= 64u) ? ~0ull : ((1ull << hi) - 1ull);
    return up & ~((1ull << lo) - 1ull);
}

template <int K, int CT, int RB>
__global__ __launch_bounds__(WAVE, CT <= 16 ? 2 : LS_WAVES_PER_SIMD) void linesearch_ndcg_kernel(LSArgs a) {
    extern __shared__ __attribute__((aligned(16))) double wdyn[];
    __shared__ double tr[RB * LS_ROWPAD];
    __shared__ double thr[WAVE];
    __shared__ double cwl[WAVE];
    __shared__ uint32_t rowcls[RB];
    const uint32_t lane = threadIdx.x;
    uint32_t g, q, q1, pos, run_end, first_lo = 0, cand0 = 0;
    if (a.work_list != nullptr) {
        const uint32_t e = blockIdx.x >> 2, sl = blockIdx.x & 3u;
        if (a.work_count != nullptr && e >= *a.work_count) return;
        const uint32_t entry = a.work_list[e];
        if (((entry >> sl) & 1u) == 0u) return;
        cand0 = sl * 16u;
        const uint32_t item = entry >> 4;
        g = item % a.G;
        q = item / a.G;
        q1 = q + 1;
        const uint32_t qs = a.qstart[q];
        pos = qs;
        run_end = qs + a.qlen[q];
    } else {
        const uint32_t blk = blockIdx.x;
        const uint32_t xcd = blk & 7u, seq = blk >> 3;
        g = a.g_base + seq % a.G;
        const uint32_t ri = (seq / a.G) * 8u + xcd;
        if (ri >= a.nruns) return;
        const uint32_t r = a.run_order[ri];
        q = a.run_q0[r];
        q1 = a.run_q1[r];
        pos = a.run_pos[r];
        first_lo = a.run_lo[r];
        run_end = pos + a.run_docs[r];
    }
    const uint32_t f = a.gfeat[g];
    const uint32_t ncand_all = a.gncand[g];
    const uint32_t ncand = ncand_all > cand0 ? (ncand_all - cand0 < (uint32_t)CT ? ncand_all - cand0 : (uint32_t)CT) : 0u;
    if (ncand == 0u) return;
    if (a.work_list != nullptr && a.slice_count != nullptr && lane == 0) atomicAdd(a.slice_count, 1u);
    const uint32_t dq = a.dq, dp = a.dq * 4, d = a.d;
    const double* __restrict__ w = a.gw + (size_t)g * dp;
    const double NEG_INF = -__builtin_huge_val();
    double* wpre = wdyn;
    double* wsuf = wdyn + dp;
    for (uint32_t j = lane; j < dp; j += WAVE) {
        const double wv = j < d ? w[j] : 0.0;
        wpre[j] = j < f ? wv : 0.0;
        wsuf[j] = j > f ? wv : 0.0;
    }
    thr[lane] = NEG_INF;
    cwl[lane] = a.gcand[(size_t)g * 64 + (cand0 + lane < 64u ? cand0 + lane : 63u)];
    __syncthreads();

    double slot_s[K];
    uint32_t slot_c[K];
#pragma unroll
    for (int m = 0; m < K; m++) {
        slot_s[m] = NEG_INF;
        slot_c[m] = 0;
    }
    bool nan_seen = false;
    uint32_t dbg_rows = 0, dbg_batches = 0, dbg_ins = 0;
    const uint64_t lt_mask = (lane == 0) ? 0ull : (~0ull >> (64 - lane));
    uint32_t qn = a.qlen[q];
    uint32_t q_end = pos + first_lo + qn;
    const uint32_t ngp = (f + 3) >> 2;
    const uint32_t sq0 = (f + 1) >> 2;
    const uint32_t fgrp = f >> 2, fsub = f & 3;

    constexpr int LS_RING = 8;
    float4 xq[CT <= 16 ? LS_RING : 1];
    const uint32_t dq_ring = (dq + (uint32_t)LS_RING - 1u) / (uint32_t)LS_RING * (uint32_t)LS_RING;
    uint32_t ld_pb = pos, ld_e = 0;
    size_t ld_base = 0;
#define LS_RING_BASE()                                                                     \
    {                                                                                      \
        const uint32_t lp_ = ld_pb + lane < a.np ? ld_pb + lane : a.np - 1u;               \
        ld_base = (size_t)(lp_ >> 6) * dq * 64 + (lp_ & 63u);                              \
    }
#define LS_RING_LOAD(DST)                                                                  \
    {                                                                                      \
        DST = a.xb[ld_base + (size_t)(ld_e < dq ? ld_e : dq - 1u) * 64];                   \
        if (++ld_e == dq_ring) {                                                           \
            ld_e = 0;                                                                      \
            if (ld_pb + (uint32_t)WAVE < run_end) ld_pb += (uint32_t)WAVE;                 \
            LS_RING_BASE()                                                                 \
        }                                                                                  \
    }
    if constexpr (CT <= 16) {
        LS_RING_BASE()
#pragma unroll
        for (int u = 0; u < LS_RING; u++) LS_RING_LOAD(xq[u])
    }
    for (uint32_t pb = pos; pb < run_end; pb += WAVE) {
        double sc[CT];
        uint32_t mycls;
        if constexpr (CT <= 16) {
            mycls = a.gcls[pb + lane < a.np ? pb + lane : a.np - 1u];
            double P = 0.0;
            for (uint32_t j0 = 0; j0 < dq_ring; j0 += (uint32_t)LS_RING) {
#pragma unroll
                for (int u = 0; u < LS_RING; u++) {
                    const uint32_t j4 = j0 + (uint32_t)u;
                    const float4 cur = xq[u];
                    if (j4 < dq) {
                        if (j4 < ngp) {
                            const double* wp = wpre + j4 * 4;
                            double p0 = (double)cur.x * wp[0];
                            P = P + p0;
                            double p1 = (double)cur.y * wp[1];
                            P = P + p1;
                            double p2 = (double)cur.z * wp[2];
                            P = P + p2;
                            double p3 = (double)cur.w * wp[3];
                            P = P + p3;
                        }
                        if (j4 == fgrp) {
                            const double xf = (double)(fsub == 0 ? cur.x : (fsub == 1 ? cur.y : (fsub == 2 ? cur.z : cur.w)));
#pragma unroll
                            for (int c = 0; c < CT; c++) {
                                double prod = xf * cwl[c];
                                sc[c] = P + prod;
// ... 167 lines not shown
```

fastrank_amd/csrc/kernels_order.inc:

```
constexpr uint32_t WT = WALK_TILE;
constexpr uint32_t WT_DPL = WT / 64;

__device__ __forceinline__ void order_segment(uint32_t s, uint32_t idx, uint32_t len, uint32_t* lo, uint32_t* hi) {
    *lo = s & 0xFFu;
    *hi = s >> 8;
    if (idx >= len || *hi <= *lo) {
        *lo = idx;
        *hi = idx + 1u;
    }
}

constexpr int ORDER_OQ = 2;
__global__ __launch_bounds__(WAVE) void xslot_kernel(const float4* __restrict__ xb, const uint16_t* __restrict__ seg, const uint32_t* __restrict__ wt_start,
                                                     uint32_t np, uint32_t dq, uint32_t d, uint8_t* __restrict__ out) {
    __shared__ float4 xs[ORDER_OQ][WT];
    const uint32_t lane = threadIdx.x;
    const uint32_t pb = wt_start[blockIdx.x];
    const uint32_t len = min(wt_start[blockIdx.x + 1] - pb, WT);
    const uint32_t j0 = blockIdx.y * ORDER_OQ;
    uint32_t lo[WT_DPL], hi[WT_DPL];
    float4 mine[WT_DPL][ORDER_OQ];
#pragma unroll
    for (uint32_t h = 0; h < WT_DPL; h++) {
        const uint32_t idx = lane + 64u * h;
        const uint32_t p = pb + (idx < len ? idx : 0u);
        order_segment(seg[p], idx, len, &lo[h], &hi[h]);
#pragma unroll
        for (int u = 0; u < ORDER_OQ; u++) {
            const uint32_t j4 = j0 + u < dq ? j0 + u : dq - 1;
            const float4 v = xb[((size_t)(p >> 6) * dq + j4) * 64 + (p & 63u)];
            const float ninf = -__builtin_huge_valf();
            mine[h][u] = make_float4(v.x == v.x ? v.x : ninf, v.y == v.y ? v.y : ninf, v.z == v.z ? v.z : ninf, v.w == v.w ? v.w : ninf);
            xs[u][idx] = mine[h][u];
        }
    }
    __syncthreads();
#pragma unroll
    for (uint32_t h = 0; h < WT_DPL; h++) {
        const uint32_t idx = lane + 64u * h;
        if (idx >= len) continue;
        uint32_t r[ORDER_OQ][4];
#pragma unroll
        for (int u = 0; u < ORDER_OQ; u++)
#pragma unroll
            for (int k = 0; k < 4; k++) r[u][k] = 0;
        for (uint32_t i = lo[h]; i < hi[h]; i++) {
            const bool before = i < idx;
#pragma unroll
            for (int u = 0; u < ORDER_OQ; u++) {
                const float4 o = xs[u][i];
                r[u][0] += (o.x > mine[h][u].x) || (o.x == mine[h][u].x && before);
                r[u][1] += (o.y > mine[h][u].y) || (o.y == mine[h][u].y && before);
                r[u][2] += (o.z > mine[h][u].z) || (o.z == mine[h][u].z && before);
                r[u][3] += (o.w > mine[h][u].w) || (o.w == mine[h][u].w && before);
            }
        }
#pragma unroll
        for (int u = 0; u < ORDER_OQ; u++)
#pragma unroll
            for (int k = 0; k < 4; k++) {
                const uint32_t f = (j0 + u) * 4 + k;
                if (j0 + u < dq && f < d) out[(size_t)f * np + pb + idx] = (uint8_t)(lo[h] + r[u][k]);
            }
    }
}

__global__ __launch_bounds__(WAVE) void xcol_kernel(const float4* __restrict__ xb, uint32_t np, uint32_t dq, uint32_t d, float* __restrict__ out) {
    const uint32_t lane = threadIdx.x, tile = blockIdx.x;
    const size_t p = (size_t)tile * 64u + lane;
    const uint32_t j0 = blockIdx.y * ORDER_OQ;
    float4 v[ORDER_OQ];
#pragma unroll
    for (int u = 0; u < ORDER_OQ; u++) v[u] = xb[((size_t)tile * dq + (j0 + u < dq ? j0 + u : dq - 1)) * 64 + lane];
#pragma unroll
    for (int u = 0; u < ORDER_OQ; u++) {
        const uint32_t f = (j0 + u) * 4;
        if (j0 + u < dq) {
            if (f + 0 < d) out[(size_t)(f + 0) * np + p] = v[u].x;
            if (f + 1 < d) out[(size_t)(f + 1) * np + p] = v[u].y;
            if (f + 2 < d) out[(size_t)(f + 2) * np + p] = v[u].z;
            if (f + 3 < d) out[(size_t)(f + 3) * np + p] = v[u].w;
        }
    }
}

template <uint32_t J, uint32_t KK, uint32_t HI>
__device__ __forceinline__ uint32_t order_exchange(uint32_t key, uint32_t lane) {
    constexpr uint64_t keep_min = [] {
        uint64_t m = 0;
        for (uint32_t l = 0; l < 64; l++) {
            const uint32_t e = l + 64u * HI;
            const bool up = (e & KK) == 0u, lower = (e & J) == 0u;
            if (up == lower) m |= 1ull << l;
        }
        return m;
    }();
    const uint32_t other = (uint32_t)__builtin_amdgcn_ds_bpermute((int)((lane ^ J) << 2), (int)key);
    const uint32_t mn = key < other ? key : other, mx = key < other ? other : key;
    return ((keep_min >> lane) & 1ull) ? mn : mx;
}
template <uint32_t KK, uint32_t HI>
__device__ __forceinline__ uint32_t order_merge(uint32_t key, uint32_t lane) {
    if constexpr (KK >= 64) key = order_exchange<32, KK, HI>(key, lane);
    if constexpr (KK >= 32) key = order_exchange<16, KK, HI>(key, lane);
    if constexpr (KK >= 16) key = order_exchange<8, KK, HI>(key, lane);
    if constexpr (KK >= 8) key = order_exchange<4, KK, HI>(key, lane);
    if constexpr (KK >= 4) key = order_exchange<2, KK, HI>(key, lane);
    return order_exchange<1, KK, HI>(key, lane);
}
static_assert(WT == 128, "the sort below is the 128-element network (two registers per lane)");
constexpr uint32_t RSLOT_BATCH = 4;
__global__ __launch_bounds__(256) void rslot_kernel(const double* __restrict__ res, const int32_t* __restrict__ slot_half,
                                                     const int32_t* __restrict__ slot_group, uint32_t nlist, const double* __restrict__ rs_par,
                                                     const uint32_t* __restrict__ rs_updf, const float* __restrict__ xcol,
                                                     const uint16_t* __restrict__ seg, const uint32_t* __restrict__ wt_start,
                                                     const uint32_t* __restrict__ wlist, uint32_t nw, uint32_t np, uint8_t* __restrict__ out) {
    const uint32_t lane = threadIdx.x & 63u, wi = blockIdx.x * 4u + (threadIdx.x >> 6);
    if (wi >= nw) return;
    const uint32_t ti = wlist ? wlist[wi] : wi;
    const uint32_t pb = wt_start[ti];
    const uint32_t len = min(wt_start[ti + 1] - pb, WT);
    uint32_t p[2], sidx[2];
    {
        uint32_t lo0, hi0, lo1, hi1;
        p[0] = pb + (lane < len ? lane : 0u);
        p[1] = pb + (lane + 64u < len ? lane + 64u : 0u);
        order_segment(seg[p[0]], lane, len, &lo0, &hi0);
        order_segment(seg[p[1]], lane + 64u, len, &lo1, &hi1);
        const uint64_t s0 = __ballot(lo0 == lane), s1 = __ballot(lo1 == lane + 64u);
        const uint64_t upto = (lane >= 63u) ? ~0ull : ((2ull << lane) - 1ull);
        sidx[0] = (uint32_t)__popcll(s0 & upto) - 1u;
        sidx[1] = (uint32_t)__popcll(s0) + (uint32_t)__popcll(s1 & upto) - 1u;
    }
    for (uint32_t k0 = 0; k0 < nlist; k0 += RSLOT_BATCH) {
        float r[RSLOT_BATCH][2];
        int32_t sh[RSLOT_BATCH];
#pragma unroll
        for (uint32_t u = 0; u < RSLOT_BATCH; u++) {
            const uint32_t k = k0 + u < nlist ? k0 + u : nlist - 1;
            sh[u] = slot_half[k];
            double R0 = res[(size_t)sh[u] * np + p[0]], R1 = res[(size_t)sh[u] * np + p[1]];
            const double* par = rs_par + (size_t)slot_group[k] * 6;
            if (par[2] != 0.0) {
                const float* xu = xcol + (size_t)rs_updf[slot_group[k]] * np;
                const double x0 = (double)xu[p[0]], x1 = (double)xu[p[1]];
                R0 = __builtin_fma(x0, par[5], __builtin_fma(-x0, par[4], R0 * par[3]));
                R1 = __builtin_fma(x1, par[5], __builtin_fma(-x1, par[4], R1 * par[3]));
            }
            r[u][0] = (float)R0;
            r[u][1] = (float)R1;
        }
#pragma unroll
        for (uint32_t u = 0; u < RSLOT_BATCH; u++) {
            if (k0 + u >= nlist) break;
            uint32_t key[2];
#pragma unroll
            for (uint32_t h = 0; h < 2; h++) {
                const uint32_t bits = __float_as_uint(r[u][h] == r[u][h] ? r[u][h] : -__builtin_huge_valf());
                const uint32_t mono = bits ^ ((uint32_t)((int32_t)bits >> 31) | 0x80000000u);
                key[h] = (sidx[h] << 25) | ((~mono >> 14) << 7) | (lane + 64u * h);
            }
            key[0] = order_merge<2, 0>(key[0], lane), key[1] = order_merge<2, 1>(key[1], lane);
            key[0] = order_merge<4, 0>(key[0], lane), key[1] = order_merge<4, 1>(key[1], lane);
            key[0] = order_merge<8, 0>(key[0], lane), key[1] = order_merge<8, 1>(key[1], lane);
            key[0] = order_merge<16, 0>(key[0], lane), key[1] = order_merge<16, 1>(key[1], lane);
            key[0] = order_merge<32, 0>(key[0], lane), key[1] = order_merge<32, 1>(key[1], lane);
            key[0] = order_merge<64, 0>(key[0], lane), key[1] = order_merge<64, 1>(key[1], lane);
            {
                const uint32_t mn = key[0] < key[1] ? key[0] : key[1], mx = key[0] < key[1] ? key[1] : key[0];
                key[0] = mn, key[1] = mx;
            }
            key[0] = order_merge<64, 0>(key[0], lane);
            key[1] = order_merge<64, 0>(key[1], lane);
#pragma unroll
            for (uint32_t h = 0; h < 2; h++) {
                const uint32_t from = key[h] & 127u;
                if (from < len) out[(size_t)(sh[u] >> 1) * np + pb + from] = (uint8_t)(lane + 64u * h);
            }
        }
    }
}

__global__ void rslot_identity_kernel(uint8_t* __restrict__ out, const uint8_t* __restrict__ wofs, size_t np, size_t n) {
    for (size_t i = (size_t)blockIdx.x * blockDim.x + threadIdx.x; i < n; i += (size_t)gridDim.x * blockDim.x) out[i] = wofs[i % np];
}

__global__ __launch_bounds__(256) void order_audit_kernel(const uint8_t* __restrict__ table, const uint16_t* __restrict__ seg,
                                                           const uint32_t* __restrict__ wt_start, const uint32_t* __restrict__ wlist, uint32_t nw,
                                                           unsigned long long* bad) {
    __shared__ uint32_t hits[4][WT];
    const uint32_t lane = threadIdx.x & 63u, w = threadIdx.x >> 6, wi = blockIdx.x * 4u + w;
    const bool on = wi < nw;
    const uint32_t ti = on ? (wlist ? wlist[wi] : wi) : 0u;
    const uint32_t pb = wt_start[ti];
    const uint32_t len = on ? min(wt_start[ti + 1] - pb, WT) : 0u;
    for (uint32_t h = 0; h < WT_DPL; h++) hits[w][lane + 64u * h] = 0u;
    __syncthreads();
    unsigned long long mine = 0;
    for (uint32_t h = 0; h < WT_DPL; h++) {
        const uint32_t idx = lane + 64u * h;
        if (idx >= len) continue;
        const uint16_t s = seg[pb + idx];
        const uint32_t lo = s & 0xFFu, hi = s >> 8;
        if (hi <= lo) continue;
        const uint32_t slot = table[pb + idx];
        if (slot < lo || slot >= hi) mine++;
        else atomicAdd(&hits[w][slot], 1u);
    }
    __syncthreads();
    for (uint32_t h = 0; h < WT_DPL; h++) {
        const uint32_t idx = lane + 64u * h;
        if (idx >= len) continue;
        const uint16_t s = seg[pb + idx];
        if ((s >> 8) > (s & 0xFFu) && hits[w][idx] != 1u) mine++;
    }
    if (mine) atomicAdd(bad, mine);
}

struct ColStats {
    double sum, sumsq;
    float mn, mx;
    unsigned long long at_min, at_max;
};
__global__ __launch_bounds__(256) void colstats_kernel(const float4* __restrict__ xb, const uint16_t* __restrict__ seg, uint32_t ntiles, uint32_t dq,
                                                       uint32_t d, int pass, ColStats* __restrict__ st) {
    const uint32_t lane = threadIdx.x & 63u, w = threadIdx.x >> 6, j4 = blockIdx.y;
    double s[4] = {0, 0, 0, 0}, s2[4] = {0, 0, 0, 0};
    float mn[4], mx[4];
    unsigned long long cmin[4] = {0, 0, 0, 0}, cmax[4] = {0, 0, 0, 0};
    float emin[4], emax[4];
#pragma unroll
    for (int k = 0; k < 4; k++) {
        mn[k] = __builtin_huge_valf();
        mx[k] = -__builtin_huge_valf();
        const uint32_t f = j4 * 4 + k;
        emin[k] = (pass == 1 && f < d) ? st[f].mn : 0.0f;
        emax[k] = (pass == 1 && f < d) ? st[f].mx : 0.0f;
    }
    for (uint32_t t = blockIdx.x * 4 + w; t < ntiles; t += gridDim.x * 4) {
        const uint16_t sg = seg[(size_t)t * 64 + lane];
        if ((sg >> 8) <= (sg & 0xFF)) continue;
        const float4 v = xb[((size_t)t * dq + j4) * 64 + lane];
        const float x[4] = {v.x, v.y, v.z, v.w};
#pragma unroll
        for (int k = 0; k < 4; k++) {
            if (pass == 0) {
                s[k] += (double)x[k];
                s2[k] += (double)x[k] * (double)x[k];
                mn[k] = x[k] < mn[k] ? x[k] : mn[k];
                mx[k] = x[k] > mx[k] ? x[k] : mx[k];
            } else {
                cmin[k] += x[k] == emin[k];
                cmax[k] += x[k] == emax[k];
            }
        }
    }
#pragma unroll
    for (int k = 0; k < 4; k++) {
        const uint32_t f = j4 * 4 + k;
        if (f >= d) continue;
        if (pass == 0) {
            atomicAdd(&st[f].sum, s[k]);
            atomicAdd(&st[f].sumsq, s2[k]);
            const float lo = mn[k] + 0.0f, hi = mx[k] + 0.0f;
            if (lo >= 0.0f) atomicMin(reinterpret_cast<int*>(&st[f].mn), __float_as_int(lo));
            else atomicMax(reinterpret_cast<unsigned int*>(&st[f].mn), __float_as_uint(lo));
            if (hi >= 0.0f) atomicMax(reinterpret_cast<int*>(&st[f].mx), __float_as_int(hi));
            else atomicMin(reinterpret_cast<unsigned int*>(&st[f].mx), __float_as_uint(hi));
        } else {
            if (cmin[k]) atomicAdd(&st[f].at_min, cmin[k]);
            if (cmax[k]) atomicAdd(&st[f].at_max, cmax[k]);
        }
    }
}
```

fastrank_amd/csrc/kernels_verify.inc:

```

__device__ __forceinline__ uint32_t verify_key_sign(uint32_t hi) { return (uint32_t)((int32_t)hi >> 31); }
#define VERIFY_BITS_SRC(WZ, VB) (DUP ? ((WZ) ^ verify_key_sign((uint32_t)((VB) >> 32))) : (WZ))
__device__ __forceinline__ bool verify_far(double ka, double kb, double eps0, double gam) {
    return (ka - kb) > __builtin_fma(gam, __builtin_fabs(ka) + __builtin_fabs(kb), eps0);
}
#ifndef VERIFY_ADMIT
#define VERIFY_ADMIT(C) (__ballot(C) != 0ull)
#endif
#ifndef VERIFY_CHAIN_PARTS
#define VERIFY_CHAIN_PARTS 3
#endif
#define VERIFY_PAIRS(GI, LO, HI)                                                                               \
                _Pragma("unroll") for (int m = (LO); m < (HI); m++) {                                          \
                    double down_;                                                                              \
                    asm("v_min_f64 %0, %1, %2\n\tv_max_f64 %1, %1, %2" : "=&v"(down_), "+v"(slot[GI][m]) : "v"(carry_)); \
                    carry_ = down_;                                                                            \
                }
#define VERIFY_CHAINS(GI)                                                                                      \
            constexpr int T1_ = VERIFY_CHAIN_PARTS == 3 ? KS / 3 : 0, T2_ = VERIFY_CHAIN_PARTS == 3 ? (2 * KS) / 3 : KS / 2; \
            if constexpr (K >= 10 && !DUP) {                                                                   \
                if (VERIFY_ADMIT(key_ >= slot[GI][T2_ - 1])) {                                                   \
                    if constexpr (T1_ > 0) {                                                                   \
                        if (VERIFY_ADMIT(key_ >= slot[GI][T1_ > 0 ? T1_ - 1 : 0])) verify_chain<(T1_ > 0 ? T1_ : 2), false, KS, 0>(slot[GI], carry_); \
                    }                                                                                          \
                    verify_chain<T2_ - T1_, false, KS, T1_>(slot[GI], carry_);                                  \
                }                                                                                              \
                verify_chain<KS - T2_, true, KS, T2_>(slot[GI], carry_);                                       \
            } else {                                                                                           \
                if (VERIFY_ADMIT(key_ >= slot[GI][T2_ - 1])) {                                                   \
                    if constexpr (T1_ > 0) {                                                                   \
                        if (VERIFY_ADMIT(key_ >= slot[GI][T1_ > 0 ? T1_ - 1 : 0])) { VERIFY_PAIRS(GI, 0, T1_) }   \
                    }                                                                                          \
                    VERIFY_PAIRS(GI, T1_, T2_)                                                                 \
                }                                                                                              \
                VERIFY_PAIRS(GI, T2_, KS - 1)                                                                  \
                asm("v_max_f64 %0, %0, %1" : "+v"(slot[GI][KS - 1]) : "v"(carry_));                            \
            }
#define VERIFY_VISIT(GI, W)                                                                                    \
    {                                                                                                          \
        const double Ad_ = __longlong_as_double((long long)(((uint64_t)(W).y << 32) | (W).x));                 \
        const double xf_ = __longlong_as_double((long long)(((uint64_t)(W).w << 32) | (W).z));                 \
        const double v_ = __builtin_fma(xf_, cw[GI], Ad_);                                                     \
        if (VERIFY_ADMIT(v_ >= slot[GI][KS - 1])) {                                                              \
            nchain++;                                                             \
                                                                        \
            const uint64_t vb_ = (uint64_t)__double_as_longlong(v_);                                           \
            uint32_t lo_;       \
            asm("v_bfi_b32 %0, %1, %2, %3" : "=v"(lo_) : "s"(cls_mask), "v"(VERIFY_BITS_SRC((W).z, vb_)), "v"((uint32_t)vb_)); \
            const double key_ = __longlong_as_double((long long)((vb_ & 0xFFFFFFFF00000000ull) | lo_));        \
            double carry_ = key_;                                                                              \
            VERIFY_CHAINS(GI)                                                                                  \
        }                                                                                                      \
    }

#define VERIFY_CE(S, i, j)                                                                                     \
    {                                                                                                          \
        double lo_;                                                                                            \
        asm("v_min_f64 %0, %1, %2\n\tv_max_f64 %1, %1, %2" : "=&v"(lo_), "+v"(S[i]) : "v"(S[j]));             \
        S[j] = lo_;                                                                                            \
    }
#include "kernels_fillnet.inc"
template <int KS> __device__ __forceinline__ void verify_fill_sort(double (&s)[KS]) {
    if constexpr (KS == 6) { VERIFY_FILL_SORT_6(s) }
    else if constexpr (KS == 7) { VERIFY_FILL_SORT_7(s) }
    else if constexpr (KS == 8) { VERIFY_FILL_SORT_8(s) }
    else if constexpr (KS == 9) { VERIFY_FILL_SORT_9(s) }
    else if constexpr (KS == 11) { VERIFY_FILL_SORT_11(s) }
    else if constexpr (KS == 12) { VERIFY_FILL_SORT_12(s) }
    else if constexpr (KS == 13) { VERIFY_FILL_SORT_13(s) }
    else if constexpr (KS == 14) { VERIFY_FILL_SORT_14(s) }
    else if constexpr (KS == 21) { VERIFY_FILL_SORT_21(s) }
    else if constexpr (KS == 22) { VERIFY_FILL_SORT_22(s) }
    else if constexpr (KS == 23) { VERIFY_FILL_SORT_23(s) }
    else { static_assert(KS == 24, "verify_fill_sort: no network of this size"); VERIFY_FILL_SORT_24(s) }
}
#define VERIFY_KEY(W, OUT)                                                                                     \
    {                                                                                                          \
        const double v_ = __builtin_fma(__longlong_as_double((long long)(((uint64_t)(W).w << 32) | (W).z)), cw[0], \
                                        __longlong_as_double((long long)(((uint64_t)(W).y << 32) | (W).x)));   \
        const uint64_t vb_ = (uint64_t)__double_as_longlong(v_);                                               \
        uint32_t lo_;                                                                                          \
        asm("v_bfi_b32 %0, %1, %2, %3" : "=v"(lo_) : "s"(cls_mask), "v"(VERIFY_BITS_SRC((W).z, vb_)), "v"((uint32_t)vb_)); \
        OUT = __longlong_as_double((long long)((vb_ & 0xFFFFFFFF00000000ull) | lo_));                          \
    }

#ifndef VERIFY_LIVE_ONLY
#define VERIFY_LIVE_ONLY(L) (L)
#endif
#ifndef VERIFY_RANK_BARRIER
#define VERIFY_RANK_BARRIER __builtin_amdgcn_sched_barrier(0);
#endif
#ifndef VERIFY_RES_WAVES
#define VERIFY_RES_WAVES 7
#endif
#ifndef VERIFY_RES_WAVES_LONG
#define VERIFY_RES_WAVES_LONG 7
#endif
#ifndef VERIFY_RES_WAVES_20
#define VERIFY_RES_WAVES_20 6
#endif
#ifndef VERIFY_RES_WAVES_20_LONG
#define VERIFY_RES_WAVES_20_LONG 5
#endif

template <int K, int GW, bool RESIDENT, int XS = 1, bool DUP = false>
__global__ __launch_bounds__(WAVE, (RESIDENT && GW == 1) ? (K >= 20 ? (XS > 1 ? VERIFY_RES_WAVES_20_LONG : VERIFY_RES_WAVES_20) : (XS > 2 ? VERIFY_RES_WAVES_LONG : VERIFY_RES_WAVES)) : (GW >= 4 ? 2 : ((K >= 20 && GW == 2) ? 3 : 4)))
void linesearch_verify_kernel(LSArgs a) {
    constexpr int KS = K + XS;
    constexpr uint32_t VT = RESIDENT ? WT : (uint32_t)WAVE;
    constexpr uint32_t DPL = VT / (uint32_t)WAVE;
    extern __shared__ __attribute__((aligned(16))) double wl[];
    __shared__ __attribute__((aligned(16))) uint4 pk[RESIDENT ? 2 : GW][VT + 4];
    const uint32_t lane = threadIdx.x;
    double* const dtab = wl + (RESIDENT ? 0u : (uint32_t)GW * a.dq * 4u);
    const uint32_t ts = a.ncls + 1u;
    for (uint32_t c = lane; c < ts; c += WAVE)
#pragma unroll
        for (int r = 0; r <= K; r++) dtab[(uint32_t)r * ts + c] = (r < K && c < a.ncls) ? a.dcgtab[(size_t)c * LS_KT + r] : 0.0;
    const uint32_t nb = (a.G + GW - 1) / GW;
    const uint32_t blk = blockIdx.x;
    const uint32_t xcd = blk & 7u, seq = blk >> 3;
    const uint32_t g0 = (seq % nb) * GW;
    const uint32_t ri = (seq / nb) * 8u + xcd;
    if (ri >= a.nruns) return;
    const uint32_t r = a.run_order[ri];
    uint32_t q = a.run_q0[r];
    const uint32_t q1 = a.run_q1[r];
    const uint32_t pos = a.run_pos[r];
    const uint32_t first_lo = a.run_lo[r];
    const uint32_t run_end = pos + a.run_docs[r];
    const uint32_t dq = a.dq, dp = a.dq * 4, d = a.d;
    const double NEG_INF = -__builtin_huge_val();
    const uint32_t cls_mask = a.cls_mask;
    uint32_t f[GW];
    bool live[GW], redo[GW], qbad[GW];
    double cw[GW], my_eps2[GW], slot[GW][KS];
    double *rcur[GW], *roth[GW];
    double r_inv[GW], r_basef[GW], u_inv[GW], u_basef[GW], u_cand[GW];
    bool r_upd[GW];
    uint32_t u_f[GW];
    const double* par_g = nullptr;
#pragma unroll
    for (int gi = 0; gi < GW; gi++) {
        const uint32_t g = g0 + gi < a.G ? g0 + gi : a.G - 1;
        f[gi] = a.gfeat[g];
        live[gi] = (g0 + gi < a.G) && lane < a.gncand[g];
        cw[gi] = a.gcand[(size_t)g * 64 + lane];
        my_eps2[gi] = a.eps2[(size_t)g * 64 + lane];
        redo[gi] = false;
        if constexpr (RESIDENT) {
            const int32_t sl = a.rs_slot[g];
            rcur[gi] = a.res_cur + (size_t)sl * a.np;
            roth[gi] = a.res_cur + (size_t)(sl ^ 1) * a.np;
            const double* par = a.rs_par + (size_t)g * 6;
            par_g = par;
            r_inv[gi] = par[0];
            r_basef[gi] = par[1];
            r_upd[gi] = par[2] != 0.0;
            u_inv[gi] = par[3];
            u_basef[gi] = par[4];
            u_cand[gi] = par[5];
            u_f[gi] = a.rs_updf[g];
        } else {
            const double* __restrict__ w = a.gw + (size_t)g * dp;
            for (uint32_t j = lane; j < dp; j += WAVE) wl[gi * dp + j] = (j < d && j != f[gi]) ? w[j] : 0.0;
        }
#pragma unroll
        for (int m = 0; m < KS; m++) slot[gi][m] = live[gi] ? NEG_INF : __builtin_huge_val();
    }
    uint32_t lbase = 0;
    bool lminus = false;
    if constexpr (RESIDENT) {
        static_assert(!RESIDENT || GW == 1, "the resident variants take one group per wave");
        if (a.xslot != nullptr) {
            const uint32_t g = g0 < a.G ? g0 : a.G - 1;
            const double delta = cw[0] - r_basef[0];
            const uint32_t mode = a.gmode[g];
            const bool near = !live[0] || !(__builtin_fabs(delta) >= a.gthr[g]) || (delta > 0.0 ? (mode & 1u) != 0u : (mode & 2u) != 0u);
            lminus = !near && delta < 0.0;
            lbase = near ? 0u : (uint32_t)sizeof(pk[0]);
        }
    }
    __syncthreads();
    uint32_t qn = a.qlen[q];
    uint32_t q_end = pos + first_lo + qn;
    bool fresh = true;
    uint32_t nchain = 0;
    uint32_t wti = 0, pb = pos, lo_first = first_lo;
    if constexpr (RESIDENT) {
        wti = a.run_wt0[r];
        pb = a.wt_start[wti];
        lo_first = pos + first_lo - pb;
    }
    bool first_tile = true;

    while (pb < run_end) {
        uint32_t pb_next = pb + (uint32_t)WAVE;
        if constexpr (RESIDENT) pb_next = a.wt_start[++wti];
        const uint32_t nvalid = (run_end < pb_next ? run_end : pb_next) - pb;
        const uint32_t lo_tile = first_tile ? lo_first : 0u;
        const float4* __restrict__ tile = RESIDENT ? nullptr : a.xb + (size_t)(pb >> 6) * dq * 64 + lane;
        float xf_res[RESIDENT ? DPL : GW];
        double A[RESIDENT ? DPL : GW];
        uint32_t mycls[DPL], i0[DPL], i1[DPL];
        if constexpr (RESIDENT) {
            constexpr int gi = 0;
            double t_inv, t_basef, tu_inv, tu_basef, tu_cand;
            {
                {
                    typedef uint32_t u32x4 __attribute__((ext_vector_type(4)));
                    typedef uint32_t u32x8 __attribute__((ext_vector_type(8)));
                    u32x4 p4;
                    u32x8 p8;
                    asm volatile("s_load_dwordx4 %0, %2, 0x0\n\ts_load_dwordx8 %1, %2, 0x10\n\ts_waitcnt lgkmcnt(0)"
                                 : "=&s"(p4), "=&s"(p8) : "s"(par_g));
                    t_inv = __longlong_as_double((long long)(((uint64_t)p4.y << 32) | p4.x));
                    t_basef = __longlong_as_double((long long)(((uint64_t)p4.w << 32) | p4.z));
                    tu_inv = __longlong_as_double((long long)(((uint64_t)p8.w << 32) | p8.z));
                    tu_basef = __longlong_as_double((long long)(((uint64_t)p8.s5 << 32) | p8.s4));
                    tu_cand = __longlong_as_double((long long)(((uint64_t)p8.s7 << 32) | p8.s6));
                }
            }
            const uint32_t rslot_row = (uint32_t)a.rs_slot[g0 < a.G ? g0 : a.G - 1] >> 1;
#pragma unroll
            for (uint32_t h = 0; h < DPL; h++) {
                const uint32_t idx = lane + 64u * h;
                const bool mine = idx >= lo_tile && idx < nvalid;
                const uint32_t p = pb + (idx < nvalid ? idx : 0u);
                double R = rcur[gi][p];
                if (r_upd[gi]) {
                    const double xu = (double)a.xcol[(size_t)u_f[gi] * a.np + p];
                    R = __builtin_fma(xu, tu_cand, __builtin_fma(-xu, tu_basef, R * tu_inv));
                    if (mine) roth[gi][p] = R;
                }
                xf_res[h] = a.xcol[(size_t)f[gi] * a.np + p];
                A[h] = __builtin_fma(-(double)xf_res[h], t_basef, R * t_inv);
                mycls[h] = a.gkey[p];
                i0[h] = i1[h] = idx;
                if (a.xslot != nullptr) {
                    i0[h] = a.rslot[(size_t)rslot_row * a.np + p];
                    i1[h] = a.xslot[(size_t)f[gi] * a.np + p];
                }
            }
        } else {
#pragma unroll
        for (int gi = 0; gi < GW; gi++) A[gi] = 0.0;
        for (uint32_t j4 = 0; j4 < dq; j4 += 8) {
            float4 xa[8];
#pragma unroll
            for (int u = 0; u < 8; u++) xa[u] = tile[(size_t)(j4 + u < dq ? j4 + u : dq - 1) * 64];
#pragma unroll
            for (int u = 0; u < 8; u++) {
                if (j4 + u < dq) {
                    const double x0 = (double)xa[u].x, x1 = (double)xa[u].y, x2 = (double)xa[u].z, x3 = (double)xa[u].w;
#pragma unroll
                    for (int gi = 0; gi < GW; gi++) {
                        const double* wp = wl + gi * dp + (j4 + u) * 4;
                        A[gi] = __builtin_fma(x0, wp[0], A[gi]);
                        A[gi] = __builtin_fma(x1, wp[1], A[gi]);
                        A[gi] = __builtin_fma(x2, wp[2], A[gi]);
                        A[gi] = __builtin_fma(x3, wp[3], A[gi]);
                    }
                }
            }
        }
        }
        if constexpr (!RESIDENT) mycls[0] = a.gkey[pb + lane];
        __syncthreads();
        if constexpr (RESIDENT) {
#pragma unroll
            for (uint32_t h = 0; h < DPL; h++) {
                const uint32_t idx = lane + 64u * h;
                redo[0] |= (idx >= lo_tile && idx < nvalid) && !(__builtin_fabs(A[h]) < 1e300);
                const uint64_t Ab = (uint64_t)__double_as_longlong(A[h]);
                const uint64_t Xb = (uint64_t)__double_as_longlong((double)xf_res[h]) | mycls[h];
                const uint4 word = make_uint4((uint32_t)Ab, (uint32_t)(Ab >> 32), (uint32_t)Xb, (uint32_t)(Xb >> 32));
                if (idx < nvalid) {
                    pk[0][i0[h] & (VT - 1u)] = word;
                    pk[1][i1[h] & (VT - 1u)] = word;
                }
            }
        } else {
#pragma unroll
        for (int gi = 0; gi < GW; gi++) {
            const float xf = ((const float*)(tile + (size_t)(f[gi] >> 2) * 64))[f[gi] & 3];
            redo[gi] |= !(__builtin_fabs(A[gi]) < 1e300);
            const uint64_t Ab = (uint64_t)__double_as_longlong(A[gi]);
            const uint64_t Xb = (uint64_t)__double_as_longlong((double)xf) | mycls[0];
            pk[gi][lane] = make_uint4((uint32_t)Ab, (uint32_t)(Ab >> 32), (uint32_t)Xb, (uint32_t)(Xb >> 32));
        }
        }
        __syncthreads();
        uint32_t lo = lo_tile;
        while (lo < nvalid) {
            const uint32_t seg_hi = (q_end - pb) < nvalid ? (q_end - pb) : nvalid;
            if constexpr (RESIDENT) {
                const char* const pkb = reinterpret_cast<const char*>(&pk[0][0]) + lbase;
                if (VERIFY_LIVE_ONLY(live[0])) {
                uint32_t flo = lo, bhi = seg_hi;
                if (fresh && seg_hi - lo >= (uint32_t)KS && !(LS_DEBUG(a) & 1)) {
                    uint32_t fa = (lminus ? seg_hi - 4u : lo) << 4;
                    const uint32_t fstep = lminus ? 0xFFFFFFC0u : 64u;
                    double fk[KS];
#pragma unroll
                    for (int i = 0; i + 4 <= KS; i += 4) {
                        const uint4 w0 = *reinterpret_cast<const uint4*>(pkb + fa), w1 = *reinterpret_cast<const uint4*>(pkb + fa + 16),
                                    w2 = *reinterpret_cast<const uint4*>(pkb + fa + 32), w3 = *reinterpret_cast<const uint4*>(pkb + fa + 48);
                        VERIFY_KEY(w0, fk[i])
                        VERIFY_KEY(w1, fk[i + 1])
                        VERIFY_KEY(w2, fk[i + 2])
                        VERIFY_KEY(w3, fk[i + 3])
                        fa += fstep;
                    }
                    if constexpr ((KS & 3) != 0) {
                        const uint32_t ta = lminus ? fa + (uint32_t)((4 - (KS & 3)) << 4) : fa;
                        const uint4 w0 = *reinterpret_cast<const uint4*>(pkb + ta);
                        VERIFY_KEY(w0, fk[KS & ~3])
                        if constexpr ((KS & 3) > 1) {
                            const uint4 w1 = *reinterpret_cast<const uint4*>(pkb + ta + 16);
                            VERIFY_KEY(w1, fk[(KS & ~3) + 1])
                        }
                        if constexpr ((KS & 3) > 2) {
                            const uint4 w2 = *reinterpret_cast<const uint4*>(pkb + ta + 32);
                            VERIFY_KEY(w2, fk[(KS & ~3) + 2])
                        }
                    }
                    verify_fill_sort<KS>(fk);
#pragma unroll
                    for (int m = 0; m < KS; m++) slot[0][m] = live[0] ? fk[m] : __builtin_huge_val();
                    flo = lo + (uint32_t)KS;
                    bhi = seg_hi - (uint32_t)KS;
                }
                const uint32_t n = (LS_DEBUG(a) & 1) ? 0u : seg_hi - flo, J = n >> 2, rem = n & 3u;
                uint32_t addr = (lminus ? bhi - 4u : flo) << 4;
                const uint32_t step = lminus ? 0xFFFFFFC0u : 64u;
                for (uint32_t j = 0; j < J; j++) {
                    const uint4 w0 = *reinterpret_cast<const uint4*>(pkb + addr), w1 = *reinterpret_cast<const uint4*>(pkb + addr + 16),
                                w2 = *reinterpret_cast<const uint4*>(pkb + addr + 32), w3 = *reinterpret_cast<const uint4*>(pkb + addr + 48);
                    VERIFY_VISIT(0, w0)
                    VERIFY_VISIT(0, w1)
                    VERIFY_VISIT(0, w2)
                    VERIFY_VISIT(0, w3)
                    addr += step;
                }
                if (rem != 0u) {
                    const uint32_t ta = (lminus ? lo : flo + (J << 2)) << 4;
                    const uint4 w0 = *reinterpret_cast<const uint4*>(pkb + ta), w1 = *reinterpret_cast<const uint4*>(pkb + ta + 16),
                                w2 = *reinterpret_cast<const uint4*>(pkb + ta + 32);
                    VERIFY_VISIT(0, w0)
                    if (rem > 1u) VERIFY_VISIT(0, w1)
                    if (rem > 2u) VERIFY_VISIT(0, w2)
                }
                }
                fresh = false;
            } else {
#pragma unroll
            for (int gi = 0; gi < GW; gi++) {
                for (uint32_t L = (LS_DEBUG(a) & 1) ? seg_hi : lo; L < seg_hi; L += 4) {
                    const uint4 w0 = pk[gi][L], w1 = pk[gi][L + 1], w2 = pk[gi][L + 2], w3 = pk[gi][L + 3];
                    VERIFY_VISIT(gi, w0)
                    if (L + 1 < seg_hi) VERIFY_VISIT(gi, w1)
                    if (L + 2 < seg_hi) VERIFY_VISIT(gi, w2)
                    if (L + 3 < seg_hi) VERIFY_VISIT(gi, w3)
                }
            }
            }
            if (q_end - pb > nvalid) break;
            const double norm = a.norms[q];
            const double gam = a.gamma;
            const uint32_t Ld = (uint32_t)a.depth < qn ? (uint32_t)a.depth : qn;
#pragma unroll
            for (int gi = 0; gi < GW; gi++) {
                if (live[gi]) {
                    double dcg = 0.0;
                    bool ok = true;
                    if constexpr (DUP) {
                        const uint32_t cmask = a.cls_only_mask, dmask = cls_mask & ~a.cls_only_mask;
                        bool allSame = true, allDup = true;
#pragma unroll
                        for (int i = 0; i < K; i++) {
                            if ((uint32_t)i < Ld) {
                                const double hi = slot[gi][i], nx = slot[gi][i + 1];
                                const uint64_t hraw = (uint64_t)__double_as_longlong(hi), nraw = (uint64_t)__double_as_longlong(nx);
                                const uint64_t hb = hraw ^ (uint64_t)(verify_key_sign((uint32_t)(hraw >> 32)) & cls_mask);
                                const uint64_t nb = nraw ^ (uint64_t)(verify_key_sign((uint32_t)(nraw >> 32)) & cls_mask);
                                const uint32_t cls = (uint32_t)hb & cmask;
                                const double term = dtab[(uint32_t)i * ts + cls];
                                dcg = dcg + term;
                                ok &= (hi < __builtin_huge_val());
                                if ((uint32_t)(i + 1) < qn) {
                                    const bool real = nx > NEG_INF;
                                    const bool far = verify_far(hi, nx, my_eps2[gi], gam) & real;
                                    const bool same = (((uint32_t)nb & cmask) == cls) & real;
                                    const bool dupp = real & (((hb ^ nb) & ~(uint64_t)cmask) == 0ull) & (((uint32_t)hb & dmask) != 0u);
                                    allSame = far | (allSame & same);
                                    allDup = far | (allDup & dupp);
                                    if ((uint32_t)(i + 1) < Ld) {
                                        ok &= allSame | allDup;
                                    } else if constexpr (XS == 1) {
                                        ok &= far;
                                    } else {
                                        bool okc = far, cs = allSame, cd = allDup;
#pragma unroll
                                        for (int t = 1; t < XS; t++) {
                                            const double ka = slot[gi][i + t], kb = slot[gi][i + t + 1];
                                            const uint64_t kar = (uint64_t)__double_as_longlong(ka), kbr = (uint64_t)__double_as_longlong(kb);
                                            const uint64_t kab = kar ^ (uint64_t)(verify_key_sign((uint32_t)(kar >> 32)) & cls_mask);
                                            const uint64_t kbb = kbr ^ (uint64_t)(verify_key_sign((uint32_t)(kbr >> 32)) & cls_mask);
                                            const bool real_t = kb > NEG_INF;
                                            const bool far_t = ((uint32_t)(i + t + 1) >= qn) | (verify_far(ka, kb, my_eps2[gi], gam) & real_t);
                                            okc |= (cs | cd) & far_t;
                                            cs &= (((uint32_t)kbb & cmask) == cls) & real_t;
                                            cd &= real_t & (((kab ^ kbb) & ~(uint64_t)cmask) == 0ull) & (((uint32_t)kab & dmask) != 0u);
                                        }
                                        ok &= okc;
                                    }
                                }
                            }
                        }
                    } else {
                        const uint32_t cmask_plain = a.cls_only_mask;
                        if constexpr (XS == 1) {
                            ok = slot[gi][0] < __builtin_huge_val();
#pragma unroll
                            for (int i = 0; i < K; i++) {
                                const bool counts = (uint32_t)i < Ld;
                                const uint32_t lo_i = (uint32_t)__double_as_longlong(slot[gi][i]);
                                const uint32_t lo_n = (uint32_t)__double_as_longlong(slot[gi][i + 1]);
                                const uint32_t roff = (counts ? (uint32_t)i : (uint32_t)K) * ts;
                                const double term = dtab[roff + (lo_i & cmask_plain)];
                                const bool need = counts && (uint32_t)(i + 1) < qn;
                                const bool incut = (uint32_t)(i + 1) < Ld;
                                const bool far = verify_far(slot[gi][i], slot[gi][i + 1], my_eps2[gi], gam);
                                const bool same = ((lo_i ^ lo_n) & cmask_plain) == 0u;
                                ok &= !need | far | (incut & same);
                                dcg = dcg + term;
                                if constexpr (K <= 10) { VERIFY_RANK_BARRIER }
                            }
                        } else {
    #pragma unroll
                        for (int i = 0; i < K; i++) {
                            if ((uint32_t)i < Ld) {
                                const double hi = slot[gi][i], nx = slot[gi][i + 1];
                                const uint32_t cls = (uint32_t)__double_as_longlong(hi) & cmask_plain;
                                double term = dtab[(uint32_t)i * ts + cls];
                                dcg = dcg + term;
                                ok &= (hi < __builtin_huge_val());
                                if ((uint32_t)(i + 1) < qn) {
                                    const bool far = verify_far(hi, nx, my_eps2[gi], gam) & (nx > NEG_INF);
                                    const bool same = (((uint32_t)__double_as_longlong(nx) & cmask_plain) == cls) & (nx > NEG_INF);
                                    if ((uint32_t)(i + 1) < Ld) {
                                        ok &= far | same;
                                    } else {
                                        bool okc = far, chain = same;
    #pragma unroll
                                        for (int t = 1; t < XS; t++) {
                                            const double ka = slot[gi][i + t], kb = slot[gi][i + t + 1];
                                            const bool far_t = ((uint32_t)(i + t + 1) >= qn) | (verify_far(ka, kb, my_eps2[gi], gam) & (kb > NEG_INF));
                                            okc |= chain & far_t;
                                            chain &= (((uint32_t)__double_as_longlong(kb) & cmask_plain) == cls) & (kb > NEG_INF);
                                        }
                                        ok &= okc;
                                    }
                                }
                            }
                        }
                        }
                    }
                    double val = 0.0;
                    if (norm == norm) {
                        if (ok && dcg > norm) atomicOr(a.flags, FLAG_ACTUAL_GT_IDEAL);
                        val = dcg / norm;
                    }
                    a.M[(size_t)q * a.ldm + (size_t)(g0 + gi) * 64 + lane] = val;
                    qbad[gi] = !ok && !(LS_DEBUG(a) & 1);
                } else {
                    qbad[gi] = false;
                }
            }
#pragma unroll
            for (int gi = 0; gi < GW; gi++) {
                const uint64_t bad = __ballot(qbad[gi]) | (__ballot(redo[gi]) != 0ull ? ~0ull : 0ull);
                if (g0 + gi < a.G && bad != 0ull && lane == 0) {
                    const uint32_t sm = ((bad & 0xFFFFull) ? 1u : 0u) | ((bad & 0xFFFF0000ull) ? 2u : 0u) | ((bad & 0xFFFF00000000ull) ? 4u : 0u) |
                                        ((bad >> 48) ? 8u : 0u);
                    uint32_t* const cnt = reinterpret_cast<uint32_t*>(a.redo_count);
                    a.redo_list[atomicAdd(cnt, 1u)] = (q * a.G + g0 + gi) * 16u + sm;
                    atomicAdd(cnt + 4 + g0 + gi, 1u);
                }
            }
            lo = seg_hi;
            q++;
            if (q >= q1) break;
#pragma unroll
            for (int gi = 0; gi < GW; gi++)
#pragma unroll
                for (int m = 0; m < KS; m++) slot[gi][m] = live[gi] ? NEG_INF : __builtin_huge_val();
            qn = a.qlen[q];
            q_end += qn;
            fresh = true;
        }
        pb = pb_next;
        first_tile = false;
    }
    if (a.chain_count != nullptr && lane == 0 && nchain != 0u && g0 < a.G) atomicAdd(a.chain_count + g0, nchain);
}
#undef VERIFY_VISIT

__global__ void resident_update_kernel(LSArgs a) {
    const uint32_t g = a.g_base + blockIdx.y;
    const double* par = a.rs_par + (size_t)g * 6;
    if (par[2] == 0.0) return;
    const uint32_t p = posmap_position(a.posmap);
    if (p == IDX_INVALID) return;
    const int32_t sl = a.rs_slot[g];
    const uint32_t uf = a.rs_updf[g];
    const double xu = (double)a.xcol[(size_t)uf * a.np + p];
    const double R = a.res_cur[(size_t)sl * a.np + p];
// ... 10 lines not shown
```

fastrank_amd/native.py:

```python
import ctypes as C
import json
import math
from typing import Dict, List, Optional, Tuple

import numpy as np

from .clib import ALLREDUCE_SUM_FN, CDataset, CModel, CQRel, HistTreeOptions, _json_reply, _load, _status, _take_str, _unwrap


def device_count() -> int:
    return int(_load().fr_device_count())


def set_device(ordinal: int) -> None:
    if _load().fr_set_device(int(ordinal)) != 0:
        raise RuntimeError("fr_set_device({}) failed".format(ordinal))


def version() -> str:
    return _load().fr_version().decode("utf-8")


def synchronize() -> None:
    if _load().fr_synchronize() != 0:
# ... 266 lines not shown
    numbers = np.zeros(6, dtype=np.int32)
    _status(
        _load().fr_debug_hist_quantise(
            dataset.pointer, lam.ctypes.data, wt.ctypes.data, lam.shape[0], int(bits), int(seed), int(tree),
            None if qs is None else qs.ctypes.data, 0 if qs is None else len(qs), 0 if goss is None else 1, float(top_rate), float(other_rate),
            int(goss_seed), int(goss_tree), q.ctypes.data, w.ctypes.data, n, C.byref(n_out), numbers.ctypes.data,
        )
    )
    names = ("s_l", "s_w", "search_s_l", "search_s_w", "d", "d_w")
    out = {k: int(v) for k, v in zip(names, numbers)}
    out["q"], out["w"] = q[: n_out.value].astype(np.int64), w[: n_out.value].astype(np.int64)
    return out


def hist_root_histogram(dataset: CDataset, lam: np.ndarray, wt: np.ndarray, split_candidates: int, quant=None, features=None):
    lam = np.ascontiguousarray(lam, dtype=np.float64)
    wt = np.ascontiguousarray(wt, dtype=np.float64)
    if lam.shape != wt.shape or lam.ndim != 1:
        raise ValueError("lam and wt must be 1-d arrays of the same length")
    bits, seed, tree = (0, 0, 0) if quant is None else (int(x) for x in quant)
    if quant is not None and not 2 <= bits <= 8:
        raise ValueError("quant bits must be between 2 and 8")
    fs = None if features is None else np.ascontiguousarray(features, dtype=np.uint32)
    F = len(dataset.feature_ids()) if fs is None else len(fs)
    k = int(split_candidates)
    cnt = np.zeros(F * k, dtype=np.uint32)
    qs = np.zeros(F * k, dtype=np.int64)
    ws = np.zeros(F * k, dtype=np.int64)
    _status(
        _load().fr_debug_hist_root_histogram(
            dataset.pointer, lam.ctypes.data, wt.ctypes.data, lam.shape[0], k, bits, seed, tree, None if fs is None else fs.ctypes.data,
            0 if fs is None else len(fs), cnt.ctypes.data, qs.ctypes.data, ws.ctypes.data, F * k,
        )
    )
    return cnt.astype(np.int64).reshape(F, k), qs.reshape(F, k), ws.reshape(F, k)


def rank_order(model: CModel, dataset: CDataset) -> Tuple[np.ndarray, np.ndarray]:
    nq = num_queries(dataset)
    n = int(_load().fr_dataset_num_instances(dataset.pointer))
    ids = np.zeros(n, dtype=np.uint32)
    offs = np.zeros(nq + 1, dtype=np.uint64)
    _status(_load().fr_rank_order(model.pointer, dataset.pointer, ids.ctypes.data, n, offs.ctypes.data, nq + 1))
    return ids, offs


def evaluate_candidates(dataset: CDataset, evaluator: str, features, base_weights, candidates: List,
                        qrel: Optional[CQRel] = None, per_query: bool = False):
    G = len(features)
    feats = np.ascontiguousarray(features, dtype=np.uint32)
    base = np.ascontiguousarray(base_weights, dtype=np.float64)
    assert base.ndim == 2 and base.shape[0] == G
    ncand = np.asarray([len(c) for c in candidates], dtype=np.uint32)
    cand = np.zeros((G, 64), dtype=np.float64)
    for g, c in enumerate(candidates):
        cand[g, : len(c)] = c
    means = np.zeros((G, 64), dtype=np.float64)
    pq = np.zeros((num_queries(dataset), G * 64), dtype=np.float64) if per_query else None
    _status(
        _load().fr_evaluate_candidates(
            dataset.pointer, None if qrel is None else qrel.pointer, evaluator.encode("utf-8"), G,
            feats.ctypes.data, base.ctypes.data, ncand.ctypes.data, cand.ctypes.data, means.ctypes.data,
            None if pq is None else pq.ctypes.data,
        )
    )
    out = [means[g, : ncand[g]].copy() for g in range(G)]
    return (out, pq) if per_query else out


def profile_enable(on: bool = True) -> None:
    _load().fr_profile_enable(1 if on else 0)


def profile_reset() -> None:
    _load().fr_profile_reset()


def profile_stats() -> Dict[str, Dict[str, float]]:
    rows = _json_reply(_load().fr_profile_json())
    return {
        r["kernel"]: {"launches": r["launches"], "total_ms": r["total_ms"],
                      "avg_ms": r["total_ms"] / max(1, r["launches"])}
        for r in rows
    }


def last_train_stats() -> Dict:
    return _json_reply(_load().fr_last_train_stats())


def last_tree_plan() -> Dict:
    return _json_reply(_load().fr_debug_tree_plan())


def train_model_shard(dataset: CDataset, train_req, restart_begin: int, restart_end: int) -> Dict:
    request = json.dumps(train_req.to_dict()).encode("utf-8")
    return _json_reply(_load().fr_train_model_shard(request, dataset.pointer, restart_begin, restart_end))


class CoordinateAscentRun:

    def __init__(self, dataset: CDataset, train_req, restart_begin: int = 0, restart_end: Optional[int] = None):
        if restart_end is None:
            restart_end = int(train_req.params.num_restarts)
        err = C.c_void_p()
        request = json.dumps(train_req.to_dict()).encode("utf-8")
        self.pointer = _load().fr_ca_begin(request, dataset.pointer, restart_begin, restart_end, C.byref(err))
        if not self.pointer:
            _status(err.value)
            raise RuntimeError("fr_ca_begin failed")
        self._dataset = dataset
        self.finished = False

    def step(self, ticks: int) -> int:
        done = C.c_uint64(0)
        fin = C.c_int(0)
        _status(_load().fr_ca_step(self.pointer, int(ticks), C.byref(done), C.byref(fin)))
        self.finished = bool(fin.value)
        return int(done.value)

    def state(self) -> Dict:
        return _json_reply(_load().fr_ca_state(self.pointer))

    def capture(self, on: bool = True) -> None:
        _status(_load().fr_ca_capture(self.pointer, 1 if on else 0))

    def take_capture(self) -> List[Dict]:
        L = _load()
        head = _json_reply(L.fr_ca_capture_take(self.pointer, None, None, 0))
        blob = np.zeros(int(head["bytes"]), dtype=np.uint8)
        _json_reply(L.fr_ca_capture_take(self.pointer, b"blob", blob.ctypes.data if blob.size else None, blob.nbytes))

        def arr(ref, dtype):
            dt = np.dtype(dtype)
            return np.frombuffer(blob, dtype=dt, count=int(ref["n"]), offset=int(ref["off"])).copy()

        out = []
        for ev in head["events"]:
            if ev["type"] == "store":
                out.append({"type": "store", "slot": int(ev["slot"]), "v": arr(ev["v"], np.float64)})
                continue
            groups = []
            for g in ev["groups"]:
                par = arr(g["params"], np.float64)
                groups.append({"feature": int(g["feature"]), "weights": arr(g["weights"], np.float64),
                               "candidates": arr(g["candidates"], np.float64), "resident_slot": int(g["resident_slot"]),
                               "resident_owner": int(g["resident_owner"]), "has_update": bool(g["has_update"]),
                               "upd_feature": int(g["upd_feature"]), "resident_norm": float(par[0]),
                               "resident_base_f": float(par[1]), "resident_err": float(par[2]), "upd_norm": float(par[3]),
                               "upd_base_f": float(par[4]), "upd_cand": float(par[5])})
            inst = dict(ev["inst"])
            if "classes" in inst:
                inst["classes"] = arr(inst["classes"], np.uint32).reshape(-1, 3).tolist()
            nq, ldm, npos = int(ev["nq"]), int(ev["ldm"]), int(ev["np"])
            slots = arr(ev["res_slots"], np.int32)
            res = arr(ev["res"], np.float64).reshape(len(slots), npos) if len(slots) else np.zeros((0, npos))
            out.append({"type": "tick", "ctx": int(ev["ctx"]), "kind": ev["kind"], "measure": int(ev["measure"]),
                        "depth": int(ev["depth"]), "groups": groups, "gorder": arr(ev["gorder"], np.uint32),
                        "nverify": int(ev["nverify"]), "approx": bool(ev["approx"]), "resident": bool(ev["resident"]),
                        "ready": bool(ev["ready"]), "inst": inst, "redo": arr(ev["redo"], np.uint32),
                        "redo_groups": int(ev["redo_groups"]), "means": arr(ev["means"], np.float64),
                        "matrix": arr(ev["matrix"], np.float64).reshape(nq, ldm) if ev["has_matrix"] else None,
                        "resident_sums": {int(s): res[i] for i, s in enumerate(slots)}})
        return out

    def close(self):
        if self.pointer:
            _load().fr_ca_free(self.pointer)
            self.pointer = None

    def __del__(self):
        try:
            self.close()
        except Exception:
            pass


def rank_ordered_sum(values: "np.ndarray", group=None) -> "np.ndarray":
    import torch
    import torch.distributed as dist

    if not dist.is_available() or not dist.is_initialized() or dist.get_world_size(group) == 1:
        return np.array(values, dtype=np.float64)
    backend = dist.get_backend(group)
    dev = torch.device("cuda", torch.cuda.current_device()) if backend == "nccl" else torch.device("cpu")
    mine = torch.from_numpy(np.ascontiguousarray(values, dtype=np.float64)).to(dev)
    parts = [torch.empty_like(mine) for _ in range(dist.get_world_size(group))]
    dist.all_gather(parts, mine, group=group)
    total = parts[0].cpu().numpy().copy()
    for t in parts[1:]:
        total = total + t.cpu().numpy()
    return total


class QueryShardedRun(CoordinateAscentRun):

    def __init__(self, dataset: CDataset, train_req, total_queries: Optional[int] = None, group=None):
        local_q = num_queries(dataset)
        if total_queries is None:
            total_queries = int(rank_ordered_sum(np.array([float(local_q)]), group)[0])

        def reduce_cb(_ctx, values, n):
            try:
                arr = np.ctypeslib.as_array(values, shape=(n,))
                arr[:] = rank_ordered_sum(arr, group)
                return 0
            except Exception as exc:
                self._callback_error = exc
                return 1

        self._callback_error = None
        self._callback = ALLREDUCE_SUM_FN(reduce_cb)
        err = C.c_void_p()
        request = json.dumps(train_req.to_dict()).encode("utf-8")
        self.pointer = _load().fr_ca_begin_query_shard(request, dataset.pointer, int(total_queries), self._callback, None, C.byref(err))
        if not self.pointer:
            _status(err.value)
            raise RuntimeError("fr_ca_begin_query_shard failed")
        self._dataset = dataset
        self.finished = False
        self.total_queries = int(total_queries)


def train_model_query_sharded(dataset: CDataset, train_req, total_queries: Optional[int] = None, group=None) -> CModel:
    run = QueryShardedRun(dataset, train_req, total_queries, group)
    try:
        while not run.finished:
            run.step(1 << 20)
        restarts = run.state()["restarts"]
    finally:
        run.close()
    model = select_model(restarts, bool(train_req.params.output_ensemble))
    model.params = train_req
    return model


def select_model(restarts: List[Dict], output_ensemble: bool = False) -> CModel:
    payload = json.dumps(restarts).encode("utf-8")
    return CModel(_unwrap(_load().fr_select_model(payload, 1 if output_ensemble else 0)))


def device_plan(devices: str, device_count: int, num_restarts: int, primary_device: int = 0) -> Dict:
    return _json_reply(_load().fr_debug_device_plan(devices.encode("utf-8"), device_count, num_restarts, primary_device))


def restart_queue_replay(num_restarts: int, n_workers: int, capacity: int, lengths) -> Dict:
    arr = np.ascontiguousarray(lengths, dtype=np.uint32)
    return _json_reply(_load().fr_debug_restart_queue(int(num_restarts), int(n_workers), int(capacity), arr.ctypes.data, len(arr)))


def peer_copy(src_device: int, dst_device: int, nbytes: int = 256 << 20) -> Dict:
    return _json_reply(_load().fr_debug_peer_copy(int(src_device), int(dst_device), int(nbytes)))


def pack_restart_records(restarts: List[Dict], cap: int, dim: int) -> "np.ndarray":
    out = np.zeros((int(cap), 3 + int(dim)), dtype=np.float64)
    _status(_load().fr_pack_restart_records(json.dumps(restarts).encode("utf-8"), int(cap), int(dim), out.ctypes.data))
    return out


def unpack_restart_records(records: "np.ndarray", dim: int) -> List[Dict]:
    arr = np.ascontiguousarray(records, dtype=np.float64).reshape(-1, 3 + int(dim))
    return _json_reply(_load().fr_unpack_restart_records(arr.ctypes.data, arr.shape[0], int(dim)))


def rccl_allgather_restarts(devices: List[int], parts: List[List[Dict]]) -> Tuple[Dict, Optional[List[Dict]]]:
    n = len(devices)
    cap = max([1] + [len(p) for p in parts])
    dim = max([0] + [len(r["weights"]) for p in parts for r in p])
    blocks = np.stack([pack_restart_records(p, cap, dim) for p in parts]) if n else np.zeros((0, cap, 3 + dim))
    out = np.empty_like(blocks)
    devs = np.ascontiguousarray(devices, dtype=np.int32)
    rep = _json_reply(_load().fr_rccl_allgather(devs.ctypes.data, n, blocks.ctypes.data, cap * (3 + dim), out.ctypes.data))
    if not rep.get("ran"):
        return rep, None
    if not np.array_equal(out.view(np.uint64), blocks.view(np.uint64)):
        raise RuntimeError("rccl_allgather_restarts: rank 0's gathered records differ from the blocks the ranks contributed")
    return rep, unpack_restart_records(out, dim)


def walk_tiles(run_pos, run_q0, run_q1, qstart, qlen, np_positions: int) -> Dict:
    arrs = [np.ascontiguousarray(a, dtype=np.uint32) for a in (run_pos, run_q0, run_q1, qstart, qlen)]
    return _json_reply(_load().fr_debug_walk_tiles(arrs[0].ctypes.data, arrs[1].ctypes.data, arrs[2].ctypes.data, len(arrs[0]),
                                                   arrs[3].ctypes.data, arrs[4].ctypes.data, len(arrs[3]), int(np_positions)))


COLSTATS_DTYPE = np.dtype([("sum", "<f8"), ("sumsq", "<f8"), ("mn", "<f4"), ("mx", "<f4"), ("at_min", "<u8"), ("at_max", "<u8")])


def device_form(dataset: CDataset, slot: int = 0) -> Dict:
    L = _load()
    f = {k: int(v) for k, v in _json_reply(L.fr_debug_device_form(dataset.pointer, int(slot), None, None, 0)).items()}
    f["nonfinite"] = bool(f["nonfinite"])
    f["shares_parent_matrix"] = bool(f["shares_parent_matrix"])
    npos, dq, d, nq, nruns = f["np"], f["dq"], f["d"], f["nq"], f["nruns"]

    def table(name, dtype, count, shape=None):
        arr = np.zeros(count, dtype=dtype)
        rep = _json_reply(L.fr_debug_device_form(dataset.pointer, int(slot), name.encode("utf-8"), arr.ctypes.data, arr.nbytes))
        if not rep["present"]:
            return None
        return arr if shape is None else arr.reshape(shape)

    if f["colstats_bytes"] != COLSTATS_DTYPE.itemsize:
        raise RuntimeError("device_form: the library's ColStats record is not the one this module describes")
    f["xb"] = table("xb", np.float32, npos // 64 * dq * 256)
    f["xcol"] = table("xcol", np.float32, d * npos, (d, npos))
    f["xslot"] = table("xslot", np.uint8, d * npos, (d, npos))
    for name, dtype in (("perm", np.uint32), ("perm_host", np.uint32), ("gain", np.float32), ("gexp", np.float64), ("gcls", np.uint32),
                        ("gkey", np.uint16), ("segtab", np.uint16), ("wofs", np.uint8)):
        f[name] = table(name, dtype, npos)
    f["wt_start"] = table("wt_start", np.uint32, f["nwt"] + 1)
    f["qstart"] = table("qstart", np.uint32, nq)
    f["qlen"] = table("qlen", np.uint32, nq)
    f["qtight"] = table("qtight", np.uint32, nq + 1)
    for name in ("run_q0", "run_q1", "run_pos", "run_docs", "run_lo", "run_order", "run_wt0"):
# ... 147 lines not shown
```

Baseline: 714,000 evals/s.

## Fuse residual rank-slot refresh sort into the resident verify kernel

Result: faster. 722,400 evals/s, median of 6 (+1.2%).

```diff
diff --git a/fastrank_amd/csrc/capi.cpp b/fastrank_amd/csrc/capi.cpp
--- a/fastrank_amd/csrc/capi.cpp
+++ b/fastrank_amd/csrc/capi.cpp
@@ -1400,6 +1400,7 @@
                 inst.set("k", Value::sint(e.kbucket));
                 inst.set("xs_used", Value::sint(e.xs_used));
                 inst.set("xs_pinned", Value::boolean(e.xs_pinned));
+                inst.set("rank_slots", put(e.rank_slots));
             } else {
                 inst.set("classes", put(e.classes));
             }
@@ -1415,6 +1416,7 @@
             ev.set("matrix", put(e.matrix));
             ev.set("res_slots", put(e.res_slots));
             ev.set("res", put(e.res));
+            ev.set("rslot", put(e.rslot));
             events.push(std::move(ev));
         }
         o.set("events", std::move(events));
diff --git a/fastrank_amd/csrc/device.hpp b/fastrank_amd/csrc/device.hpp
--- a/fastrank_amd/csrc/device.hpp
+++ b/fastrank_amd/csrc/device.hpp
@@ -85,6 +85,8 @@
     std::vector<double> matrix;
     std::vector<int> res_slots;
     std::vector<double> res;
+    std::vector<uint32_t> rank_slots;
+    std::vector<uint8_t> rslot;
 };
 
 struct KernelStat {
diff --git a/fastrank_amd/csrc/device_dataset.inc b/fastrank_amd/csrc/device_dataset.inc
--- a/fastrank_amd/csrc/device_dataset.inc
+++ b/fastrank_amd/csrc/device_dataset.inc
@@ -127,6 +127,7 @@
         LsCounts counts;
         bool resident = false, dup = false;
         int kbucket = 0;
+        std::vector<uint32_t> rank_slots;
         std::vector<LineGroup> cgroups;
     };
     LsCtx ls[LS_CONTEXTS + 1];
@@ -1445,20 +1446,26 @@
     return e ? (unsigned)std::min<long>(std::max<long>(std::atol(e), 64), 1 << 20) : 0u;
 }
 
+template <int K, bool RANK>
+static void launch_verify_resident(const LSArgs& a, bool dupk, int xs, dim3 grid, size_t tab_lds, hipStream_t st) {
+    if (dupk) {
+        if (xs <= 1) linesearch_verify_kernel<K, 1, true, 1, true, RANK><<<grid, dim3(WAVE), tab_lds, st>>>(a);
+        else if (xs == 2) linesearch_verify_kernel<K, 1, true, 2, true, RANK><<<grid, dim3(WAVE), tab_lds, st>>>(a);
+        else if (xs == 3 || K < 10) linesearch_verify_kernel<K, 1, true, 3, true, RANK><<<grid, dim3(WAVE), tab_lds, st>>>(a);
+        else linesearch_verify_kernel<K, 1, true, (K < 10 ? 3 : 4), true, RANK><<<grid, dim3(WAVE), tab_lds, st>>>(a);
+    } else if (xs <= 1) linesearch_verify_kernel<K, 1, true, 1, false, RANK><<<grid, dim3(WAVE), tab_lds, st>>>(a);
+    else if (xs == 2) linesearch_verify_kernel<K, 1, true, 2, false, RANK><<<grid, dim3(WAVE), tab_lds, st>>>(a);
+    else if (xs == 3 || K < 10) linesearch_verify_kernel<K, 1, true, 3, false, RANK><<<grid, dim3(WAVE), tab_lds, st>>>(a);
+    else linesearch_verify_kernel<K, 1, true, (K < 10 ? 3 : 4), false, RANK><<<grid, dim3(WAVE), tab_lds, st>>>(a);
+}
+
 template <int K>
-static void launch_verify(const LSArgs& a, bool resident, bool dupk, int xs, unsigned nruns8, size_t G, size_t dp, size_t tab_lds_kt, hipStream_t st) {
+static void launch_verify(const LSArgs& a, bool resident, bool dupk, int xs, bool rank, unsigned nruns8, size_t G, size_t dp, size_t tab_lds_kt, hipStream_t st) {
     const size_t tab_lds = tab_lds_kt / (LS_KT + 1) * (K + 1);
     if (resident) {
         const dim3 grid((unsigned)(nruns8 * G));
-        if (dupk) {
-            if (xs <= 1) linesearch_verify_kernel<K, 1, true, 1, true><<<grid, dim3(WAVE), tab_lds, st>>>(a);
-            else if (xs == 2) linesearch_verify_kernel<K, 1, true, 2, true><<<grid, dim3(WAVE), tab_lds, st>>>(a);
-            else if (xs == 3 || K < 10) linesearch_verify_kernel<K, 1, true, 3, true><<<grid, dim3(WAVE), tab_lds, st>>>(a);
-            else linesearch_verify_kernel<K, 1, true, (K < 10 ? 3 : 4), true><<<grid, dim3(WAVE), tab_lds, st>>>(a);
-        } else if (xs <= 1) linesearch_verify_kernel<K, 1, true><<<grid, dim3(WAVE), tab_lds, st>>>(a);
-        else if (xs == 2) linesearch_verify_kernel<K, 1, true, 2><<<grid, dim3(WAVE), tab_lds, st>>>(a);
-        else if (xs == 3 || K < 10) linesearch_verify_kernel<K, 1, true, 3><<<grid, dim3(WAVE), tab_lds, st>>>(a);
-        else linesearch_verify_kernel<K, 1, true, (K < 10 ? 3 : 4)><<<grid, dim3(WAVE), tab_lds, st>>>(a);
+        if (rank) launch_verify_resident<K, true>(a, dupk, xs, grid, tab_lds, st);
+        else launch_verify_resident<K, false>(a, dupk, xs, grid, tab_lds, st);
     } else {
         const dim3 grid((unsigned)(nruns8 * ((G + 1) / 2)));
         linesearch_verify_kernel<K, 2, false><<<grid, dim3(WAVE), 2 * dp * sizeof(double) + tab_lds, st>>>(a);
@@ -2021,8 +2028,14 @@
         int32_t* rank = c.th<int32_t>(ts.o_rank);
         nrank = m.pol.plan_rank_refresh(nV, [&](size_t g) { return (size_t)groups[g].resident_slot; }, [&](size_t g) { return groups[g].has_update; },
                                         period, m.res_half, rank, rank + G);
+        for (size_t k = 0; k < nrank; k++) {
+            gmode[rank[G + k]] |= VERIFY_RANK_STORE;
+            for (size_t g = 0; g < nV; g++)
+                if (groups[g].resident_slot == (long)(rank[k] >> 1)) gmode[g] |= VERIFY_RANK_SORT;
+        }
         a.xslot = m.xslot.p;
         a.rslot = m.rslot.p;
+        a.segtab = m.segtab.p;
         a.gthr = c.td<double>(ts.o_gthr);
         a.gmode = c.td<uint32_t>(ts.o_gmode);
     }
@@ -2034,27 +2047,6 @@
             dispatch_exact(a, depth, (unsigned)(nruns8 * G), maxc, c.lds, c.stream);
         }
         return m.submit_queued(c, t, 0, err);
-    }
-    if (nrank > 0) {
-        ProfScope ps("rslot_kernel", c.stream);
-        const uint32_t* wl = m.nwlist ? m.wlist.p : nullptr;
-        const unsigned nw = (unsigned)(m.nwlist ? m.nwlist : m.nwt);
-        rslot_kernel<<<dim3((nw + 3) / 4), 256, 0, c.stream>>>(m.res.p, c.td<int32_t>(ts.o_rank), c.td<int32_t>(ts.o_rank) + G, (uint32_t)nrank,
-                                                              a.rs_par, a.rs_updf, m.xcol.p, m.segtab.p, m.wt_start.p, wl, nw, (uint32_t)m.np, m.rslot.p);
-        FR_HIP(hipGetLastError());
-        if (c.audit) {
-            if (!m.audit_cnt.ensure(1, err)) return false;
-            FR_HIP(hipMemsetAsync(m.audit_cnt.p, 0, sizeof(unsigned long long), c.stream));
-            const int32_t* rk = c.th<int32_t>(ts.o_rank);
-            for (size_t k = 0; k < nrank; k++)
-                order_audit_kernel<<<dim3((nw + 3) / 4), 256, 0, c.stream>>>(m.rslot.p + (size_t)(rk[k] >> 1) * m.np, m.segtab.p, m.wt_start.p, wl, nw, m.audit_cnt.p);
-            for (size_t g = 0; g < nV; g++)
-                order_audit_kernel<<<dim3((nw + 3) / 4), 256, 0, c.stream>>>(m.xslot.p + (size_t)groups[g].feature * m.np, m.segtab.p, m.wt_start.p, wl, nw, m.audit_cnt.p);
-            unsigned long long bad = 0;
-            FR_HIP(hipMemcpyAsync(&bad, m.audit_cnt.p, sizeof(bad), hipMemcpyDeviceToHost, c.stream));
-            FR_HIP(hipStreamSynchronize(c.stream));
-            m.audit_mismatches += bad;
-        }
     }
     const char* xs_e = frdev::path_env("FR_VERIFY_XS");
     const int xs = std::min(xs_e ? std::atoi(xs_e) : m.verify_xs, verify_xs_cap(depth));
@@ -2066,11 +2058,27 @@
     c.dup = dupk;
     {
         ProfScope ps("linesearch_verify_kernel", c.stream);
-        if (depth <= 5) launch_verify<5>(a, resident, dupk, xs, (unsigned)nruns8, nV, dp, tab_lds, c.stream), c.kbucket = 5;
-        else if (depth <= 10) launch_verify<10>(a, resident, dupk, xs, (unsigned)nruns8, nV, dp, tab_lds, c.stream), c.kbucket = 10;
-        else launch_verify<20>(a, resident, dupk, xs, (unsigned)nruns8, nV, dp, tab_lds, c.stream), c.kbucket = 20;
+        if (depth <= 5) launch_verify<5>(a, resident, dupk, xs, nrank > 0, (unsigned)nruns8, nV, dp, tab_lds, c.stream), c.kbucket = 5;
+        else if (depth <= 10) launch_verify<10>(a, resident, dupk, xs, nrank > 0, (unsigned)nruns8, nV, dp, tab_lds, c.stream), c.kbucket = 10;
+        else launch_verify<20>(a, resident, dupk, xs, nrank > 0, (unsigned)nruns8, nV, dp, tab_lds, c.stream), c.kbucket = 20;
     }
     FR_HIP(hipGetLastError());
+    c.rank_slots.clear();
+    for (size_t k = 0; k < nrank; k++) c.rank_slots.push_back((uint32_t)(c.th<int32_t>(ts.o_rank)[k] >> 1));
+    if (c.audit && nrank > 0) {
+        const uint32_t* wl = m.nwlist ? m.wlist.p : nullptr;
+        const unsigned nw = (unsigned)(m.nwlist ? m.nwlist : m.nwt);
+        if (!m.audit_cnt.ensure(1, err)) return false;
+        FR_HIP(hipMemsetAsync(m.audit_cnt.p, 0, sizeof(unsigned long long), c.stream));
+        for (uint32_t slot : c.rank_slots)
+            order_audit_kernel<<<dim3((nw + 3) / 4), 256, 0, c.stream>>>(m.rslot.p + (size_t)slot * m.np, m.segtab.p, m.wt_start.p, wl, nw, m.audit_cnt.p);
+        for (size_t g = 0; g < nV; g++)
+            order_audit_kernel<<<dim3((nw + 3) / 4), 256, 0, c.stream>>>(m.xslot.p + (size_t)groups[g].feature * m.np, m.segtab.p, m.wt_start.p, wl, nw, m.audit_cnt.p);
+        unsigned long long bad = 0;
+        FR_HIP(hipMemcpyAsync(&bad, m.audit_cnt.p, sizeof(bad), hipMemcpyDeviceToHost, c.stream));
+        FR_HIP(hipStreamSynchronize(c.stream));
+        m.audit_mismatches += bad;
+    }
     a.slice_count = c.td<uint32_t>(ts.o_count) + 1;
     const unsigned redo_pin = redo_grid_env();
     c.redo_grid_used = redo_pin ? redo_pin : c.redo_grid;
@@ -2362,7 +2370,13 @@
             const size_t slot = (size_t)e.res_slots[i];
             FR_HIP(hipMemcpyAsync(e.res.data() + i * m.np, m.res.p + (slot * 2 + m.res_half[slot]) * m.np, m.np * sizeof(double), hipMemcpyDeviceToHost, st));
         }
-    }
+        if (m.rslot.p != nullptr) {
+            e.rslot.resize(e.res_slots.size() * m.np);
+            for (size_t i = 0; i < e.res_slots.size(); i++)
+                FR_HIP(hipMemcpyAsync(e.rslot.data() + i * m.np, m.rslot.p + (size_t)e.res_slots[i] * m.np, m.np, hipMemcpyDeviceToHost, st));
+        }
+    }
+    if (c.kind == LSK_TOPK && c.kbucket) e.rank_slots = c.rank_slots;
     FR_HIP(hipStreamSynchronize(st));
     m.cap_log.push_back(std::move(e));
     return true;
diff --git a/fastrank_amd/csrc/kernels_linesearch.inc b/fastrank_amd/csrc/kernels_linesearch.inc
--- a/fastrank_amd/csrc/kernels_linesearch.inc
+++ b/fastrank_amd/csrc/kernels_linesearch.inc
@@ -39,7 +39,8 @@
     const float* xcol;
     const uint32_t* rs_updf;
     const uint8_t* xslot;
-    const uint8_t* rslot;
+    uint8_t* rslot;
+    const uint16_t* segtab;
     const double* gthr;
     const uint32_t* gmode;
     uint32_t np;
diff --git a/fastrank_amd/csrc/kernels_order.inc b/fastrank_amd/csrc/kernels_order.inc
--- a/fastrank_amd/csrc/kernels_order.inc
+++ b/fastrank_amd/csrc/kernels_order.inc
@@ -109,76 +109,39 @@
     return order_exchange<1, KK, HI>(key, lane);
 }
 static_assert(WT == 128, "the sort below is the 128-element network (two registers per lane)");
-constexpr uint32_t RSLOT_BATCH = 4;
-__global__ __launch_bounds__(256) void rslot_kernel(const double* __restrict__ res, const int32_t* __restrict__ slot_half,
-                                                     const int32_t* __restrict__ slot_group, uint32_t nlist, const double* __restrict__ rs_par,
-                                                     const uint32_t* __restrict__ rs_updf, const float* __restrict__ xcol,
-                                                     const uint16_t* __restrict__ seg, const uint32_t* __restrict__ wt_start,
-                                                     const uint32_t* __restrict__ wlist, uint32_t nw, uint32_t np, uint8_t* __restrict__ out) {
-    const uint32_t lane = threadIdx.x & 63u, wi = blockIdx.x * 4u + (threadIdx.x >> 6);
-    if (wi >= nw) return;
-    const uint32_t ti = wlist ? wlist[wi] : wi;
-    const uint32_t pb = wt_start[ti];
-    const uint32_t len = min(wt_start[ti + 1] - pb, WT);
-    uint32_t p[2], sidx[2];
+__device__ __forceinline__ void order_rank_tile(float r0, float r1, uint32_t s0, uint32_t s1, uint32_t len, uint32_t lane, uint32_t (&from)[2]) {
+    const float r[2] = {r0, r1};
+    uint32_t sidx[2];
     {
         uint32_t lo0, hi0, lo1, hi1;
-        p[0] = pb + (lane < len ? lane : 0u);
-        p[1] = pb + (lane + 64u < len ? lane + 64u : 0u);
-        order_segment(seg[p[0]], lane, len, &lo0, &hi0);
-        order_segment(seg[p[1]], lane + 64u, len, &lo1, &hi1);
-        const uint64_t s0 = __ballot(lo0 == lane), s1 = __ballot(lo1 == lane + 64u);
+        order_segment(s0, lane, len, &lo0, &hi0);
+        order_segment(s1, lane + 64u, len, &lo1, &hi1);
+        const uint64_t b0 = __ballot(lo0 == lane), b1 = __ballot(lo1 == lane + 64u);
         const uint64_t upto = (lane >= 63u) ? ~0ull : ((2ull << lane) - 1ull);
-        sidx[0] = (uint32_t)__popcll(s0 & upto) - 1u;
-        sidx[1] = (uint32_t)__popcll(s0) + (uint32_t)__popcll(s1 & upto) - 1u;
-    }
-    for (uint32_t k0 = 0; k0 < nlist; k0 += RSLOT_BATCH) {
-        float r[RSLOT_BATCH][2];
-        int32_t sh[RSLOT_BATCH];
-#pragma unroll
-        for (uint32_t u = 0; u < RSLOT_BATCH; u++) {
-            const uint32_t k = k0 + u < nlist ? k0 + u : nlist - 1;
-            sh[u] = slot_half[k];
-            double R0 = res[(size_t)sh[u] * np + p[0]], R1 = res[(size_t)sh[u] * np + p[1]];
-            const double* par = rs_par + (size_t)slot_group[k] * 6;
-            if (par[2] != 0.0) {
-                const float* xu = xcol + (size_t)rs_updf[slot_group[k]] * np;
-                const double x0 = (double)xu[p[0]], x1 = (double)xu[p[1]];
-                R0 = __builtin_fma(x0, par[5], __builtin_fma(-x0, par[4], R0 * par[3]));
-                R1 = __builtin_fma(x1, par[5], __builtin_fma(-x1, par[4], R1 * par[3]));
-            }
-            r[u][0] = (float)R0;
-            r[u][1] = (float)R1;
-        }
-#pragma unroll
-        for (uint32_t u = 0; u < RSLOT_BATCH; u++) {
-            if (k0 + u >= nlist) break;
-            uint32_t key[2];
-#pragma unroll
-            for (uint32_t h = 0; h < 2; h++) {
-                const uint32_t bits = __float_as_uint(r[u][h] == r[u][h] ? r[u][h] : -__builtin_huge_valf());
-                const uint32_t mono = bits ^ ((uint32_t)((int32_t)bits >> 31) | 0x80000000u);
-                key[h] = (sidx[h] << 25) | ((~mono >> 14) << 7) | (lane + 64u * h);
-            }
-            key[0] = order_merge<2, 0>(key[0], lane), key[1] = order_merge<2, 1>(key[1], lane);
-            key[0] = order_merge<4, 0>(key[0], lane), key[1] = order_merge<4, 1>(key[1], lane);
-            key[0] = order_merge<8, 0>(key[0], lane), key[1] = order_merge<8, 1>(key[1], lane);
-            key[0] = order_merge<16, 0>(key[0], lane), key[1] = order_merge<16, 1>(key[1], lane);
-            key[0] = order_merge<32, 0>(key[0], lane), key[1] = order_merge<32, 1>(key[1], lane);
-            key[0] = order_merge<64, 0>(key[0], lane), key[1] = order_merge<64, 1>(key[1], lane);
-            {
-                const uint32_t mn = key[0] < key[1] ? key[0] : key[1], mx = key[0] < key[1] ? key[1] : key[0];
-                key[0] = mn, key[1] = mx;
-            }
-            key[0] = order_merge<64, 0>(key[0], lane);
-            key[1] = order_merge<64, 0>(key[1], lane);
-#pragma unroll
-            for (uint32_t h = 0; h < 2; h++) {
-                const uint32_t from = key[h] & 127u;
-                if (from < len) out[(size_t)(sh[u] >> 1) * np + pb + from] = (uint8_t)(lane + 64u * h);
-            }
-        }
-    }
+        sidx[0] = (uint32_t)__popcll(b0 & upto) - 1u;
+        sidx[1] = (uint32_t)__popcll(b0) + (uint32_t)__popcll(b1 & upto) - 1u;
+    }
+    uint32_t key[2];
+#pragma unroll
+    for (uint32_t h = 0; h < 2; h++) {
+        const uint32_t bits = __float_as_uint(r[h] == r[h] ? r[h] : -__builtin_huge_valf());
+        const uint32_t mono = bits ^ ((uint32_t)((int32_t)bits >> 31) | 0x80000000u);
+        key[h] = (sidx[h] << 25) | ((~mono >> 14) << 7) | (lane + 64u * h);
+    }
+    key[0] = order_merge<2, 0>(key[0], lane), key[1] = order_merge<2, 1>(key[1], lane);
+    key[0] = order_merge<4, 0>(key[0], lane), key[1] = order_merge<4, 1>(key[1], lane);
+    key[0] = order_merge<8, 0>(key[0], lane), key[1] = order_merge<8, 1>(key[1], lane);
+    key[0] = order_merge<16, 0>(key[0], lane), key[1] = order_merge<16, 1>(key[1], lane);
+    key[0] = order_merge<32, 0>(key[0], lane), key[1] = order_merge<32, 1>(key[1], lane);
+    key[0] = order_merge<64, 0>(key[0], lane), key[1] = order_merge<64, 1>(key[1], lane);
+    {
+        const uint32_t mn = key[0] < key[1] ? key[0] : key[1], mx = key[0] < key[1] ? key[1] : key[0];
+        key[0] = mn, key[1] = mx;
+    }
+    key[0] = order_merge<64, 0>(key[0], lane);
+    key[1] = order_merge<64, 0>(key[1], lane);
+    from[0] = key[0] & 127u;
+    from[1] = key[1] & 127u;
 }
 
 __global__ void rslot_identity_kernel(uint8_t* __restrict__ out, const uint8_t* __restrict__ wofs, size_t np, size_t n) {
diff --git a/fastrank_amd/csrc/kernels_verify.inc b/fastrank_amd/csrc/kernels_verify.inc
--- a/fastrank_amd/csrc/kernels_verify.inc
+++ b/fastrank_amd/csrc/kernels_verify.inc
@@ -42,7 +42,8 @@
         const double xf_ = __longlong_as_double((long long)(((uint64_t)(W).w << 32) | (W).z));                 \
         const double v_ = __builtin_fma(xf_, cw[GI], Ad_);                                                     \
         if (VERIFY_ADMIT(v_ >= slot[GI][KS - 1])) {                                                              \
-            nchain++;                                                             \
+                                             \
+            asm("s_add_u32 %0, %0, 1" : "+s"(nrun) : : "scc");                                                  \
                                                                         \
             const uint64_t vb_ = (uint64_t)__double_as_longlong(v_);                                           \
             uint32_t lo_;       \
@@ -103,8 +104,16 @@
 #define VERIFY_RES_WAVES_20_LONG 5
 #endif
 
-template <int K, int GW, bool RESIDENT, int XS = 1, bool DUP = false>
-__global__ __launch_bounds__(WAVE, (RESIDENT && GW == 1) ? (K >= 20 ? (XS > 1 ? VERIFY_RES_WAVES_20_LONG : VERIFY_RES_WAVES_20) : (XS > 2 ? VERIFY_RES_WAVES_LONG : VERIFY_RES_WAVES)) : (GW >= 4 ? 2 : ((K >= 20 && GW == 2) ? 3 : 4)))
+#ifndef VERIFY_RANK_WAVES
+#define VERIFY_RANK_WAVES 6
+#endif
+#ifndef VERIFY_RANK_WAVES_20
+#define VERIFY_RANK_WAVES_20 5
+#endif
+
+constexpr uint32_t VERIFY_RANK_SORT = 4u, VERIFY_RANK_STORE = 8u;
+template <int K, int GW, bool RESIDENT, int XS = 1, bool DUP = false, bool RANK = false>
+__global__ __launch_bounds__(WAVE, RANK ? (K >= 20 ? VERIFY_RANK_WAVES_20 : VERIFY_RANK_WAVES) : (RESIDENT && GW == 1) ? (K >= 20 ? (XS > 1 ? VERIFY_RES_WAVES_20_LONG : VERIFY_RES_WAVES_20) : (XS > 2 ? VERIFY_RES_WAVES_LONG : VERIFY_RES_WAVES)) : (GW >= 4 ? 2 : ((K >= 20 && GW == 2) ? 3 : 4)))
 void linesearch_verify_kernel(LSArgs a) {
     constexpr int KS = K + XS;
     constexpr uint32_t VT = RESIDENT ? WT : (uint32_t)WAVE;
@@ -170,6 +179,8 @@
     }
     uint32_t lbase = 0;
     bool lminus = false;
+    uint32_t rank_bits = 0;
+    static_assert(!RANK || (RESIDENT && GW == 1), "only the resident variants refresh ranks");
     if constexpr (RESIDENT) {
         static_assert(!RESIDENT || GW == 1, "the resident variants take one group per wave");
         if (a.xslot != nullptr) {
@@ -179,6 +190,7 @@
             const bool near = !live[0] || !(__builtin_fabs(delta) >= a.gthr[g]) || (delta > 0.0 ? (mode & 1u) != 0u : (mode & 2u) != 0u);
             lminus = !near && delta < 0.0;
             lbase = near ? 0u : (uint32_t)sizeof(pk[0]);
+            if constexpr (RANK) rank_bits = (uint32_t)__builtin_amdgcn_readfirstlane((int)mode) & (VERIFY_RANK_SORT | VERIFY_RANK_STORE);
         }
     }
     __syncthreads();
@@ -203,6 +215,7 @@
         float xf_res[RESIDENT ? DPL : GW];
         double A[RESIDENT ? DPL : GW];
         uint32_t mycls[DPL], i0[DPL], i1[DPL];
+        float rsum[RANK ? DPL : 1];
         if constexpr (RESIDENT) {
             constexpr int gi = 0;
             double t_inv, t_basef, tu_inv, tu_basef, tu_cand;
@@ -233,13 +246,38 @@
                     R = __builtin_fma(xu, tu_cand, __builtin_fma(-xu, tu_basef, R * tu_inv));
                     if (mine) roth[gi][p] = R;
                 }
+                if constexpr (RANK) rsum[h] = (float)R;
                 xf_res[h] = a.xcol[(size_t)f[gi] * a.np + p];
                 A[h] = __builtin_fma(-(double)xf_res[h], t_basef, R * t_inv);
                 mycls[h] = a.gkey[p];
                 i0[h] = i1[h] = idx;
+                if constexpr (!RANK) {
                 if (a.xslot != nullptr) {
                     i0[h] = a.rslot[(size_t)rslot_row * a.np + p];
                     i1[h] = a.xslot[(size_t)f[gi] * a.np + p];
+                }
+                } else if (a.xslot != nullptr) {
+                    if (!(rank_bits & VERIFY_RANK_SORT)) i0[h] = a.rslot[(size_t)rslot_row * a.np + p];
+                    i1[h] = a.xslot[(size_t)f[gi] * a.np + p];
+                }
+            }
+            if constexpr (RANK) {
+                static_assert(!RANK || DPL == 2, "order_rank_tile ranks two documents per lane");
+                if (rank_bits & VERIFY_RANK_SORT) {
+                    __shared__ uint8_t rank_slot[WT];
+                    const uint32_t tlen = (pb_next - pb) < WT ? (pb_next - pb) : WT;
+                    const uint32_t s0 = a.segtab[pb + (lane < tlen ? lane : 0u)], s1 = a.segtab[pb + (lane + 64u < tlen ? lane + 64u : 0u)];
+                    uint32_t from[2];
+                    order_rank_tile(rsum[0], rsum[1], s0, s1, tlen, lane, from);
+#pragma unroll
+                    for (uint32_t h = 0; h < DPL; h++) {
+                        rank_slot[from[h]] = (uint8_t)(lane + 64u * h);
+                        if ((rank_bits & VERIFY_RANK_STORE) && from[h] >= lo_tile && from[h] < nvalid)
+                            a.rslot[(size_t)rslot_row * a.np + pb + from[h]] = (uint8_t)(lane + 64u * h);
+                    }
+                    __syncthreads();
+#pragma unroll
+                    for (uint32_t h = 0; h < DPL; h++) i0[h] = rank_slot[lane + 64u * h];
                 }
             }
         } else {
@@ -297,6 +335,7 @@
             if constexpr (RESIDENT) {
                 const char* const pkb = reinterpret_cast<const char*>(&pk[0][0]) + lbase;
                 if (VERIFY_LIVE_ONLY(live[0])) {
+                uint32_t nrun = 0;
                 uint32_t flo = lo, bhi = seg_hi;
                 if (fresh && seg_hi - lo >= (uint32_t)KS && !(LS_DEBUG(a) & 1)) {
                     uint32_t fa = (lminus ? seg_hi - 4u : lo) << 4;
@@ -351,9 +390,11 @@
                     if (rem > 1u) VERIFY_VISIT(0, w1)
                     if (rem > 2u) VERIFY_VISIT(0, w2)
                 }
+                nchain += nrun;
                 }
                 fresh = false;
             } else {
+            uint32_t nrun = 0;
 #pragma unroll
             for (int gi = 0; gi < GW; gi++) {
                 for (uint32_t L = (LS_DEBUG(a) & 1) ? seg_hi : lo; L < seg_hi; L += 4) {
@@ -364,6 +405,7 @@
                     if (L + 3 < seg_hi) VERIFY_VISIT(gi, w3)
                 }
             }
+            nchain += nrun;
             }
             if (q_end - pb > nvalid) break;
             const double norm = a.norms[q];
diff --git a/fastrank_amd/native.py b/fastrank_amd/native.py
--- a/fastrank_amd/native.py
+++ b/fastrank_amd/native.py
@@ -442,16 +442,21 @@
             inst = dict(ev["inst"])
             if "classes" in inst:
                 inst["classes"] = arr(inst["classes"], np.uint32).reshape(-1, 3).tolist()
+            if "rank_slots" in inst:
+                inst["rank_slots"] = arr(inst["rank_slots"], np.uint32).tolist()
             nq, ldm, npos = int(ev["nq"]), int(ev["ldm"]), int(ev["np"])
             slots = arr(ev["res_slots"], np.int32)
             res = arr(ev["res"], np.float64).reshape(len(slots), npos) if len(slots) else np.zeros((0, npos))
+            rslot = arr(ev["rslot"], np.uint8)
+            rslot = rslot.reshape(len(slots), npos) if rslot.size else None
             out.append({"type": "tick", "ctx": int(ev["ctx"]), "kind": ev["kind"], "measure": int(ev["measure"]),
                         "depth": int(ev["depth"]), "groups": groups, "gorder": arr(ev["gorder"], np.uint32),
                         "nverify": int(ev["nverify"]), "approx": bool(ev["approx"]), "resident": bool(ev["resident"]),
                         "ready": bool(ev["ready"]), "inst": inst, "redo": arr(ev["redo"], np.uint32),
                         "redo_groups": int(ev["redo_groups"]), "means": arr(ev["means"], np.float64),
                         "matrix": arr(ev["matrix"], np.float64).reshape(nq, ldm) if ev["has_matrix"] else None,
-                        "resident_sums": {int(s): res[i] for i, s in enumerate(slots)}})
+                        "resident_sums": {int(s): res[i] for i, s in enumerate(slots)},
+                        "rslot": {} if rslot is None else {int(s): rslot[i] for i, s in enumerate(slots)}})
         return out
 
     def close(self):
```
